# AndreasKarg/raytracer-weekend

Measured on AMD Instinct MI355X. Metric: Mrays/sec at 1920x1080, 512 spp, 50 bounces; 1/2/4/8-GPU scaling, higher is better.
Workload: dtype f32; 1 GPU; Random-spheres scene, 1920x1080, 512 spp, 1xMI355X (configs[1]); scene=jumpy-balls, width=1920, height=1080, spp=512, max_depth=50, rays_per_frame=3103484398, tiles=32400, launches_per_frame=1, parallelism=tiles1

## Files before the change

include/rtw.h:

```cpp
#ifndef RTW_H
#define RTW_H
#include <stddef.h>
#include <stdint.h>

#ifdef __cplusplus
extern "C" {
#endif

#define RTW_ABI_VERSION 7

enum {
  RTW_OK = 0,
  RTW_EINVAL = -22,
  RTW_ENOMEM = -12,
  RTW_ENODEV = -19,
  RTW_ESTATE = -71,
  RTW_EIO = -5
};

typedef struct rtw_scene rtw_scene;

typedef struct {
  float origin[3], lower_left_corner[3], horizontal[3], vertical[3];
  float u[3], v[3], w[3];
// ... 91 lines not shown
int rtw_progress_decode(const uint8_t* frame, size_t len, rtw_progress_msg* msg);

int rtw_render_device(rtw_scene* s, int device, const rtw_camera* cam, const float background[3],
                      uint32_t w, uint32_t h, uint32_t spp, uint32_t max_depth, uint64_t seed,
                      const uint32_t* d_tile_ids, uint32_t n_tiles, float* d_out, void* stream,
                      uint32_t flags, rtw_stats* stats);
int rtw_render_device_strided(rtw_scene* s, int device, const rtw_camera* cam, const float background[3],
                              uint32_t w, uint32_t h, uint32_t spp, uint32_t max_depth, uint64_t seed,
                              uint32_t first_tile, uint32_t tile_stride, uint32_t n_tiles, float* d_out,
                              void* stream, uint32_t flags, rtw_stats* stats);
typedef struct {
  float origin[3], direction[3];
  float time;
  uint32_t reserved;
  uint64_t stream;
} rtw_ray;
typedef struct {
  float p[3], normal[3];
  float t, u, v;
  uint32_t material, key, flags;
} rtw_hit;
enum {
  RTW_HIT_HIT = 1,
  RTW_HIT_FRONT_FACE = 2,
  RTW_HIT_BAD_RAY = 4
};
int rtw_hit_rays(rtw_scene* s, int device, uint64_t n, const void* rays, void* hits, rtw_stats* stats);
int rtw_hit_rays_device(rtw_scene* s, int device, uint64_t n, const void* d_rays, void* d_hits, void* stream,
                        rtw_stats* stats);

typedef struct {
  float attenuation[3];
  float emitted[3];
  uint32_t flags, reserved;
} rtw_scatter;
enum {
  RTW_SCATTER_SCATTERED = 1,
  RTW_SCATTER_MISS = 2,
  RTW_SCATTER_BAD = 4
};
int rtw_camera_rays(rtw_scene* s, int device, const rtw_camera* cam, uint32_t w, uint32_t h, uint32_t spp,
                    uint64_t seed, uint64_t first, uint64_t n, void* rays, rtw_stats* stats);
int rtw_camera_rays_device(rtw_scene* s, int device, const rtw_camera* cam, uint32_t w, uint32_t h, uint32_t spp,
                           uint64_t seed, uint64_t first, uint64_t n, void* d_rays, void* stream, rtw_stats* stats);
int rtw_scatter_rays(rtw_scene* s, int device, uint64_t n, const void* rays, const void* hits,
                     const float background[3], void* out_rays, void* out_scatter, rtw_stats* stats);
int rtw_scatter_rays_device(rtw_scene* s, int device, uint64_t n, const void* d_rays, const void* d_hits,
                            const float background[3], void* d_out_rays, void* d_out_scatter, void* stream,
                            rtw_stats* stats);

typedef struct {
  float color[3];
  uint32_t segments;
  uint64_t stream;
  uint32_t flags, reserved;
} rtw_sample;
enum { RTW_SAMPLE_END_MISS = 1, RTW_SAMPLE_END_NO_SCATTER = 2 ,
       RTW_SAMPLE_BAD_RAY = 4, RTW_SAMPLE_END_DEPTH = 8 };
int rtw_sample_rays(rtw_scene* s, int device, uint64_t n, const void* rays, const float background[3],
                    uint32_t max_depth, void* samples, rtw_stats* stats);
int rtw_sample_rays_device(rtw_scene* s, int device, uint64_t n, const void* d_rays, const float background[3],
                           uint32_t max_depth, void* d_samples, void* stream, rtw_stats* stats);

int rtw_render_status(rtw_scene* s, int device);
int rtw_diag_corrupt_bvh(rtw_scene* s, int device);
int rtw_diag_alias_devices(rtw_scene* s, int n);

int rtw_render_multi(rtw_scene* s, int n_gpus, const rtw_camera* cam, const float background[3], uint32_t w,
                     uint32_t h, uint32_t spp, uint32_t max_depth, uint64_t seed, float* out_rgb_sum,
                     rtw_stats* stats);
int rtw_render_multi_times(const rtw_scene* s, float* device_ms, uint32_t cap, float* gather_ms);

int rtw_tile_partition(uint32_t w, uint32_t h, uint32_t n_parts, uint32_t part, uint32_t* ids, uint32_t cap,
                       uint32_t* n_ids);

int rtw_unpack_tiles_device(int device, uint32_t w, uint32_t h, const uint32_t* d_tile_ids,
                            uint32_t n_tiles, const float* d_packed, float* d_image, void* stream);

int rtw_path_kernel_times(rtw_scene* s, int device, float* ms, uint32_t max_n);

int rtw_diag_libm(int fn, uint32_t n, const float* a, const float* b, float* out);
int rtw_diag_sweep(int fn, uint32_t lo, uint32_t hi, uint64_t* counts, uint32_t* bad, uint32_t cap);
int rtw_diag_recip(uint32_t n, const float* b, float* out);

int rtw_tonemap(const float* rgb_sum, uint32_t n_pixels, uint32_t spp, uint8_t* rgb8);

int rtw_scene_preset(rtw_scene* s, const char* name, float aspect_ratio, uint64_t seed,
                     const char* models_dir, rtw_camera* cam, float background[3]);
int rtw_preset_cameras(const char* name, float aspect_ratio, const char* models_dir, rtw_camera* cams,
                       uint32_t cap, uint32_t* n);

int rtw_scene_dump(const rtw_scene* s, char* buf, size_t cap, size_t* needed);
int rtw_scene_image(const rtw_scene* s, uint32_t k, const uint8_t** rgb8, uint32_t* w, uint32_t* h);
int64_t rtw_scene_info(const rtw_scene* s, int what);
int rtw_scene_nodes(const rtw_scene* s, const void** nodes, uint32_t* n_nodes);
int rtw_scene_nodes_half(const rtw_scene* s, const void** nodes, uint32_t* n_nodes);

#ifdef __cplusplus
}
#endif
#endif
```

raytracer-weekend_amd/__init__.py:

```python
from __future__ import annotations

import contextlib
import ctypes as C
import os
from pathlib import Path

import numpy as np

PKG_DIR = Path(__file__).resolve().parent
REPO_ROOT = PKG_DIR.parent
LIB_PATH = Path(os.environ.get("RTW_LIB_PATH") or PKG_DIR / "lib" / "librtw_amd.so")
MODELS_DIR = REPO_ROOT / "models"

RTW_EINVAL, RTW_ENOMEM, RTW_ENODEV, RTW_ESTATE, RTW_EIO = -22, -12, -19, -71, -5
FLAG_COUNT_TRAVERSAL = 1
NO_MATERIAL = 0xFFFFFFFF


class RtwError(RuntimeError):
    def __init__(self, code: int, msg: str):
        super().__init__(f"rtw error {code}: {msg}")
        self.code = code


# ... 66 lines not shown
                      ("v", np.float32), ("material", np.uint32), ("key", np.uint32), ("flags", np.uint32)])
MSG_IMAGE_START, MSG_PIXEL, MSG_IMAGE_END = 0, 1, 2
PIXEL_SINK = C.CFUNCTYPE(C.c_int, C.POINTER(rtw_pixel), C.c_uint32, C.c_void_p)
PIXEL_DTYPE = np.dtype([("row", np.uint32), ("column", np.uint32), ("color", np.float32, 3)])

_F = C.POINTER(C.c_float)
_U32 = C.POINTER(C.c_uint32)
_U8 = C.POINTER(C.c_uint8)
_SIGS = {
    "rtw_last_error": (C.c_char_p, []),
    "rtw_abi_version": (C.c_int, []),
    "rtw_device_count": (C.c_int, []),
    "rtw_scene_create": (C.c_int, [C.POINTER(C.c_void_p)]),
    "rtw_scene_destroy": (None, [C.c_void_p]),
    "rtw_texture_solid": (C.c_int, [C.c_void_p, C.c_float, C.c_float, C.c_float, _U32]),
    "rtw_texture_checker": (C.c_int, [C.c_void_p, C.c_uint32, C.c_uint32, C.c_float, _U32]),
    "rtw_texture_image": (C.c_int, [C.c_void_p, _U8, C.c_uint32, C.c_uint32, _U32]),
    "rtw_texture_uvdebug": (C.c_int, [C.c_void_p, _U32]),
    "rtw_texture_noise": (C.c_int, [C.c_void_p, _F, _U32, C.c_float, _U32]),
    "rtw_perlin_generate": (C.c_int, [C.c_uint64, _F, _U32]),
    "rtw_material_isotropic": (C.c_int, [C.c_void_p, C.c_uint32, _U32]),
    "rtw_material_lambertian": (C.c_int, [C.c_void_p, C.c_uint32, _U32]),
    "rtw_material_metal": (C.c_int, [C.c_void_p, C.c_float, C.c_float, C.c_float, C.c_float, _U32]),
    "rtw_material_dielectric": (C.c_int, [C.c_void_p, C.c_float, _U32]),
    "rtw_material_diffuse_light": (C.c_int, [C.c_void_p, C.c_uint32, _U32]),
    "rtw_begin_list": (C.c_int, [C.c_void_p]),
    "rtw_begin_bvh": (C.c_int, [C.c_void_p, C.c_float, C.c_float]),
    "rtw_begin_translate": (C.c_int, [C.c_void_p, C.c_float, C.c_float, C.c_float]),
    "rtw_begin_rotate_y": (C.c_int, [C.c_void_p, C.c_float]),
    "rtw_begin_constant_medium": (C.c_int, [C.c_void_p, C.c_float, C.c_uint32, _U32]),
    "rtw_end": (C.c_int, [C.c_void_p]),
    "rtw_add_spheres": (C.c_int, [C.c_void_p, C.c_uint32, _F, _F, _F, _F, _U32]),
    "rtw_add_moving_spheres": (C.c_int, [C.c_void_p, C.c_uint32] + [_F] * 9 + [_U32]),
    "rtw_add_rects": (C.c_int, [C.c_void_p, C.c_uint32, _U32, _F, _F, _F, _F, _F, _U32]),
    "rtw_add_cuboid": (C.c_int, [C.c_void_p, _F, _F, C.c_uint32]),
    "rtw_add_triangles": (C.c_int, [C.c_void_p, C.c_uint32, _F, _F, _U8, _F, _U8, C.c_uint32]),
    "rtw_load_wavefront_obj": (C.c_int, [C.c_void_p, C.c_char_p, C.c_void_p, C.c_uint32, _U32]),
    "rtw_scene_commit": (C.c_int, [C.c_void_p, C.c_int]),
    "rtw_camera_new": (C.c_int, [_F, _F, _F, C.c_float, C.c_float, C.c_float, C.c_float, C.c_float,
                                 C.c_float, C.POINTER(rtw_camera)]),
    "rtw_render": (C.c_int, [C.c_void_p, C.POINTER(rtw_camera), _F, C.c_uint32, C.c_uint32, C.c_uint32,
                             C.c_uint32, C.c_uint64, _F, C.POINTER(rtw_stats)]),
    "rtw_render_device": (C.c_int, [C.c_void_p, C.c_int, C.POINTER(rtw_camera), _F, C.c_uint32, C.c_uint32,
                                    C.c_uint32, C.c_uint32, C.c_uint64, _U32, C.c_uint32, C.c_void_p,
                                    C.c_void_p, C.c_uint32, C.POINTER(rtw_stats)]),
    "rtw_render_device_strided": (C.c_int, [C.c_void_p, C.c_int, C.POINTER(rtw_camera), _F, C.c_uint32,
                                            C.c_uint32, C.c_uint32, C.c_uint32, C.c_uint64, C.c_uint32, C.c_uint32,
                                            C.c_uint32, C.c_void_p, C.c_void_p, C.c_uint32, C.POINTER(rtw_stats)]),
    "rtw_hit_rays": (C.c_int, [C.c_void_p, C.c_int, C.c_uint64, C.POINTER(rtw_ray), C.POINTER(rtw_hit),
                               C.POINTER(rtw_stats)]),
    "rtw_hit_rays_device": (C.c_int, [C.c_void_p, C.c_int, C.c_uint64, C.c_void_p, C.c_void_p, C.c_void_p,
                                      C.POINTER(rtw_stats)]),
    "rtw_camera_rays": (C.c_int, [C.c_void_p, C.c_int, C.POINTER(rtw_camera), C.c_uint32, C.c_uint32, C.c_uint32,
                                  C.c_uint64, C.c_uint64, C.c_uint64, C.POINTER(rtw_ray), C.POINTER(rtw_stats)]),
    "rtw_camera_rays_device": (C.c_int, [C.c_void_p, C.c_int, C.POINTER(rtw_camera), C.c_uint32, C.c_uint32,
                                         C.c_uint32, C.c_uint64, C.c_uint64, C.c_uint64, C.c_void_p, C.c_void_p,
                                         C.POINTER(rtw_stats)]),
    "rtw_scatter_rays": (C.c_int, [C.c_void_p, C.c_int, C.c_uint64, C.POINTER(rtw_ray), C.POINTER(rtw_hit), _F,
                                   C.POINTER(rtw_ray), C.POINTER(rtw_scatter), C.POINTER(rtw_stats)]),
    "rtw_scatter_rays_device": (C.c_int, [C.c_void_p, C.c_int, C.c_uint64, C.c_void_p, C.c_void_p, _F, C.c_void_p,
                                          C.c_void_p, C.c_void_p, C.POINTER(rtw_stats)]),
    "rtw_sample_rays": (C.c_int, [C.c_void_p, C.c_int, C.c_uint64, C.POINTER(rtw_ray), _F, C.c_uint32,
                                  C.POINTER(rtw_sample), C.POINTER(rtw_stats)]),
    "rtw_sample_rays_device": (C.c_int, [C.c_void_p, C.c_int, C.c_uint64, C.c_void_p, _F, C.c_uint32, C.c_void_p,
                                         C.c_void_p, C.POINTER(rtw_stats)]),
    "rtw_render_status": (C.c_int, [C.c_void_p, C.c_int]),
    "rtw_diag_corrupt_bvh": (C.c_int, [C.c_void_p, C.c_int]),
    "rtw_diag_alias_devices": (C.c_int, [C.c_void_p, C.c_int]),
    "rtw_path_kernel_times": (C.c_int, [C.c_void_p, C.c_int, _F, C.c_uint32]),
    "rtw_render_multi": (C.c_int, [C.c_void_p, C.c_int, C.POINTER(rtw_camera), _F, C.c_uint32, C.c_uint32,
                                   C.c_uint32, C.c_uint32, C.c_uint64, _F, C.POINTER(rtw_stats)]),
    "rtw_render_multi_times": (C.c_int, [C.c_void_p, _F, C.c_uint32, _F]),
    "rtw_tile_partition": (C.c_int, [C.c_uint32, C.c_uint32, C.c_uint32, C.c_uint32, _U32, C.c_uint32, _U32]),
    "rtw_render_stream": (C.c_int, [C.c_void_p, C.POINTER(rtw_camera), _F, C.c_uint32, C.c_uint32, C.c_uint32,
                                    C.c_uint32, C.c_uint64, C.c_uint32, PIXEL_SINK, C.c_void_p,
                                    C.POINTER(rtw_stats)]),
    "rtw_progress_encode": (C.c_int, [C.POINTER(rtw_progress_msg), _U8, C.c_size_t, C.POINTER(C.c_size_t)]),
    "rtw_progress_decode": (C.c_int, [_U8, C.c_size_t, C.POINTER(rtw_progress_msg)]),
    "rtw_unpack_tiles_device": (C.c_int, [C.c_int, C.c_uint32, C.c_uint32, C.c_void_p, C.c_uint32,
                                          C.c_void_p, C.c_void_p, C.c_void_p]),
    "rtw_tonemap": (C.c_int, [_F, C.c_uint32, C.c_uint32, _U8]),
    "rtw_diag_libm": (C.c_int, [C.c_int, C.c_uint32, _F, _F, _F]),
    "rtw_diag_recip": (C.c_int, [C.c_uint32, _F, _F]),
    "rtw_diag_sweep": (C.c_int, [C.c_int, C.c_uint32, C.c_uint32, C.POINTER(C.c_uint64), _U32, C.c_uint32]),
    "rtw_scene_preset": (C.c_int, [C.c_void_p, C.c_char_p, C.c_float, C.c_uint64, C.c_char_p,
                                   C.POINTER(rtw_camera), _F]),
    "rtw_preset_cameras": (C.c_int, [C.c_char_p, C.c_float, C.c_char_p, C.POINTER(rtw_camera), C.c_uint32,
                                     _U32]),
    "rtw_scene_dump": (C.c_int, [C.c_void_p, C.c_char_p, C.c_size_t, C.POINTER(C.c_size_t)]),
    "rtw_scene_image": (C.c_int, [C.c_void_p, C.c_uint32, C.POINTER(_U8), _U32, _U32]),
    "rtw_scene_nodes": (C.c_int, [C.c_void_p, C.POINTER(C.c_void_p), _U32]),
    "rtw_scene_nodes_half": (C.c_int, [C.c_void_p, C.POINTER(C.c_void_p), _U32]),
    "rtw_scene_info": (C.c_int64, [C.c_void_p, C.c_int]),
}
EXPORTED_SYMBOLS = tuple(_SIGS)

_lib = None


ABI_VERSION = 7


def lib_sha() -> str:
    import hashlib
    return hashlib.sha256(LIB_PATH.read_bytes()).hexdigest()[:16] if LIB_PATH.exists() else ""


def lib() -> C.CDLL:
    global _lib
    if _lib is None:
        if not LIB_PATH.exists():
            raise RtwError(RTW_ENODEV, f"{LIB_PATH} not built (run __graft_entry__.build())")
        try:
            import torch
        except ImportError:
            pass
        L = C.CDLL(str(LIB_PATH))
        for name, (res, args) in _SIGS.items():
            fn = getattr(L, name)
            fn.restype = res
            fn.argtypes = args
        if L.rtw_abi_version() != ABI_VERSION:
            raise RtwError(RTW_ESTATE, f"{LIB_PATH} has ABI {L.rtw_abi_version()}, this mirror {ABI_VERSION}")
        _lib = L
    return _lib


def _check(rc: int) -> None:
    if rc != 0:
        raise RtwError(rc, lib().rtw_last_error().decode())


def _fa(x) -> np.ndarray:
    return np.ascontiguousarray(np.asarray(x, dtype=np.float32).reshape(-1))


def _ua(x) -> np.ndarray:
    return np.ascontiguousarray(np.asarray(x, dtype=np.uint32).reshape(-1))


def _fp(a: np.ndarray):
    return a.ctypes.data_as(_F)


def _up(a: np.ndarray):
    return a.ctypes.data_as(_U32)


def device_count() -> int:
    return int(lib().rtw_device_count())


class Camera:

    def __init__(self, c: rtw_camera):
        self.c = c

    @classmethod
    def new(cls, look_from, look_at, vup, vfov, aspect, aperture, focus_dist, time0=0.0, time1=1.0):
        c = rtw_camera()
        _check(lib().rtw_camera_new(_fp(_fa(look_from)), _fp(_fa(look_at)), _fp(_fa(vup)), vfov, aspect,
                                    aperture, focus_dist, time0, time1, C.byref(c)))
        return cls(c)

    def as_dict(self) -> dict:
        return {k: (list(getattr(self.c, k)) if k not in ("lens_radius", "time0", "time1")
# ... 342 lines not shown
            self.seed, first_tile, tile_stride, n_tiles, C.c_void_p(d_out_ptr), C.c_void_p(stream_ptr), flags,
            C.byref(st) if want_stats else None))
        return st.as_dict() if want_stats else None


def make_rays(origins, directions, times=None, streams=None) -> np.ndarray:
    o = np.asarray(origins, np.float32).reshape(-1, 3)
    rays = np.zeros(len(o), RAY_DTYPE)
    rays["origin"] = o
    rays["direction"] = np.asarray(directions, np.float32).reshape(-1, 3)
    if times is not None:
        rays["time"] = np.asarray(times, np.float32).reshape(-1)
    if streams is not None:
        rays["stream"] = np.asarray(streams, np.uint64).reshape(-1)
    return rays


def progress_encode(kind: int, width=0, height=0, spp=0, pixel=None) -> bytes:
    m = rtw_progress_msg(kind=kind, width=width, height=height, samples_per_pixel=spp)
    if pixel is not None:
        m.pixel.row, m.pixel.column = int(pixel[0]), int(pixel[1])
        m.pixel.color[:] = [float(x) for x in pixel[2]]
    out = (C.c_uint8 * 64)()
    n = C.c_size_t()
    _check(lib().rtw_progress_encode(C.byref(m), out, 64, C.byref(n)))
    return bytes(out[:n.value])


def progress_decode(frame: bytes) -> dict:
    buf = (C.c_uint8 * max(1, len(frame))).from_buffer_copy(frame or b"\0")
    m = rtw_progress_msg()
    _check(lib().rtw_progress_decode(buf, len(frame), C.byref(m)))
    d = {"kind": int(m.kind)}
    if m.kind == MSG_IMAGE_START:
        d.update(width=int(m.width), height=int(m.height), samples_per_pixel=int(m.samples_per_pixel))
    elif m.kind == MSG_PIXEL:
        d.update(row=int(m.pixel.row), column=int(m.pixel.column), color=[float(x) for x in m.pixel.color])
    return d


def perlin_generate(seed: int = 0):
    g = np.zeros(768, np.float32)
    p = np.zeros(768, np.uint32)
    _check(lib().rtw_perlin_generate(seed, _fp(g), _up(p)))
    return g.reshape(256, 3), p.reshape(3, 256)


def preset_cameras(name: str, aspect: float, models_dir=None) -> list:
    n = C.c_uint32()
    md = str(models_dir or MODELS_DIR).encode()
    _check(lib().rtw_preset_cameras(name.encode(), aspect, md, None, 0, C.byref(n)))
    cams = (rtw_camera * max(1, n.value))()
    _check(lib().rtw_preset_cameras(name.encode(), aspect, md, cams, n.value, C.byref(n)))
    return [Camera(cams[k]) for k in range(n.value)]


def unpack_tiles_device(w, h, d_tiles_ptr, n_tiles, d_packed_ptr, d_image_ptr, device=-1, stream_ptr=0):
    _check(lib().rtw_unpack_tiles_device(device, w, h, C.c_void_p(d_tiles_ptr), n_tiles, C.c_void_p(d_packed_ptr),
                                         C.c_void_p(d_image_ptr), C.c_void_p(stream_ptr)))


def diag_libm(fn: int, a, b=None) -> np.ndarray:
    a = _fa(a)
    bb = _fa(b) if b is not None else None
    out = np.empty_like(a)
    _check(lib().rtw_diag_libm(fn, len(a), _fp(a), _fp(bb) if bb is not None else None, _fp(out)))
    return out


def diag_sweep(fn: int, lo: int = 0, hi: int = 0xFFFFFFFF, cap: int = 64):
    counts = (C.c_uint64 * 2)()
    bad = np.zeros(max(1, cap), np.uint32)
    _check(lib().rtw_diag_sweep(fn, lo, hi, counts, _up(bad), cap))
    return int(counts[0]), int(counts[1]), bad[:min(cap, int(counts[0]))]


def diag_recip(b) -> np.ndarray:
    b = _fa(b)
    out = np.empty_like(b)
    _check(lib().rtw_diag_recip(len(b), _fp(b), _fp(out)))
    return out


def tile_partition(w: int, h: int, n_parts: int, part: int):
    nt = n_tiles(w, h)
    per = (nt + n_parts - 1) // n_parts if n_parts > 0 else 0
    ids = np.zeros(max(1, per), np.uint32)
    n = C.c_uint32()
    _check(lib().rtw_tile_partition(w, h, n_parts, part, _up(ids), per, C.byref(n)))
    return ids[:per], int(n.value)


def n_tiles(w: int, h: int) -> int:
    return ((w + 7) // 8) * ((h + 7) // 8)


def tonemap(sums: np.ndarray, spp: int) -> np.ndarray:
    s = np.ascontiguousarray(sums, np.float32)
    out = np.empty(s.shape, np.uint8)
    _check(lib().rtw_tonemap(_fp(s.reshape(-1)), s.size // 3, spp, out.ctypes.data_as(_U8)))
    return out


def image_height(width: int, aspect: float = 1.7777778) -> int:
    import math
    x = width / aspect
    return int(math.floor(x + 0.5))


def camera_aspect(width: int, height: int) -> float:
    return float(np.float32(width) / np.float32(height))
```

raytracer-weekend_amd/csrc/rtw.hpp:

```cpp
#pragma once
#include <stdexcept>
#include <string>
#include <vector>

#include "../../include/rtw.h"

namespace rtw {

struct Error : std::runtime_error {
  int code;
  Error(int c, const char* m) : std::runtime_error(m), code(c) {}
};
inline void check(int rc) {
  if (rc != RTW_OK) throw Error(rc, rtw_last_error());
}

struct Vec3 {
  float x, y, z;
};
using Point3 = Vec3;
using Color = Vec3;

struct Pixel {
  uint32_t row, column;
// ... 59 lines not shown
  World& operator=(const World&) = delete;
  rtw_scene* raw() const { return s_; }

  TextureId solid_rgb(float r, float g, float b) { TextureId t; check(rtw_texture_solid(s_, r, g, b, &t)); return t; }
  TextureId checker(TextureId odd, TextureId even, float freq) { TextureId t; check(rtw_texture_checker(s_, odd, even, freq, &t)); return t; }
  TextureId image(const uint8_t* rgb, uint32_t w, uint32_t h) { TextureId t; check(rtw_texture_image(s_, rgb, w, h, &t)); return t; }
  TextureId uv_debug() { TextureId t; check(rtw_texture_uvdebug(s_, &t)); return t; }
  TextureId noise(float scale, uint64_t perlin_seed) {
    float g[768];
    uint32_t p[768];
    check(rtw_perlin_generate(perlin_seed, g, p));
    TextureId t;
    check(rtw_texture_noise(s_, g, p, scale, &t));
    return t;
  }

  MaterialId lambertian(TextureId t) { MaterialId m; check(rtw_material_lambertian(s_, t, &m)); return m; }
  MaterialId lambertian_solid(Color c) { return lambertian(solid_rgb(c.x, c.y, c.z)); }
  MaterialId metal(Color albedo, float fuzz) { MaterialId m; check(rtw_material_metal(s_, albedo.x, albedo.y, albedo.z, fuzz, &m)); return m; }
  MaterialId dielectric(float ir) { MaterialId m; check(rtw_material_dielectric(s_, ir, &m)); return m; }
  MaterialId diffuse_light(TextureId t) { MaterialId m; check(rtw_material_diffuse_light(s_, t, &m)); return m; }
  MaterialId isotropic(TextureId t) { MaterialId m; check(rtw_material_isotropic(s_, t, &m)); return m; }

  void sphere(Point3 c, float r, MaterialId m) { check(rtw_add_spheres(s_, 1, &c.x, &c.y, &c.z, &r, &m)); }
  void moving_sphere(Point3 c0, float t0, Point3 c1, float t1, float r, MaterialId m) {
    check(rtw_add_moving_spheres(s_, 1, &c0.x, &c0.y, &c0.z, &t0, &c1.x, &c1.y, &c1.z, &t1, &r, &m));
  }
  void rect(uint32_t axis, float a0, float a1, float b0, float b1, float k, MaterialId m) {
    check(rtw_add_rects(s_, 1, &axis, &a0, &a1, &b0, &b1, &k, &m));
  }
  void xy_rect(float x0, float x1, float y0, float y1, float k, MaterialId m) { rect(0, x0, x1, y0, y1, k, m); }
  void xz_rect(float x0, float x1, float z0, float z1, float k, MaterialId m) { rect(1, x0, x1, z0, z1, k, m); }
  void yz_rect(float y0, float y1, float z0, float z1, float k, MaterialId m) { rect(2, y0, y1, z0, z1, k, m); }
  void cuboid(Point3 p0, Point3 p1, MaterialId m) {
    const float a[3] = {p0.x, p0.y, p0.z}, b[3] = {p1.x, p1.y, p1.z};
    check(rtw_add_cuboid(s_, a, b, m));
  }
  void triangle(const Point3 v[3], MaterialId m) {
    const float f[9] = {v[0].x, v[0].y, v[0].z, v[1].x, v[1].y, v[1].z, v[2].x, v[2].y, v[2].z};
    check(rtw_add_triangles(s_, 1, f, nullptr, nullptr, nullptr, nullptr, m));
  }
  uint32_t load_wavefront_obj(const std::string& path, uint32_t material_override = UINT32_MAX) {
    uint32_t n = 0;
    check(rtw_load_wavefront_obj(s_, path.c_str(), nullptr, material_override, &n));
    return n;
  }
  template <class F> void list(F&& body) { check(rtw_begin_list(s_)); body(); check(rtw_end(s_)); }
  template <class F> void bvh(float t0, float t1, F&& body) { check(rtw_begin_bvh(s_, t0, t1)); body(); check(rtw_end(s_)); }
  template <class F> void translate(Vec3 off, F&& body) { check(rtw_begin_translate(s_, off.x, off.y, off.z)); body(); check(rtw_end(s_)); }
  template <class F> void rotate_y(float deg, F&& body) { check(rtw_begin_rotate_y(s_, deg)); body(); check(rtw_end(s_)); }
  template <class F> void constant_medium(float density, TextureId t, F&& body) {
    check(rtw_begin_constant_medium(s_, density, t, nullptr)); body(); check(rtw_end(s_));
  }

  void preset(const std::string& name, float aspect, uint64_t seed, const std::string& models, Camera& cam, Color& bg) {
    float b[3];
    check(rtw_scene_preset(s_, name.c_str(), aspect, seed, models.c_str(), &cam.c, b));
    bg = Color{b[0], b[1], b[2]};
  }
  static std::vector<Camera> preset_cameras(const std::string& name, float aspect, const std::string& models) {
    uint32_t n = 0;
    check(rtw_preset_cameras(name.c_str(), aspect, models.c_str(), nullptr, 0, &n));
    std::vector<rtw_camera> raw(n);
    check(rtw_preset_cameras(name.c_str(), aspect, models.c_str(), raw.data(), n, &n));
    std::vector<Camera> out(n);
    for (uint32_t k = 0; k < n; ++k) out[k].c = raw[k];
    return out;
  }
  void commit(int device = -1) { check(rtw_scene_commit(s_, device)); }
  std::vector<Hit> hit_rays(const std::vector<Ray>& rays, int device = -1, rtw_stats* st = nullptr) const {
    std::vector<Hit> hits(rays.size());
    check(rtw_hit_rays(s_, device, rays.size(), rays.data(), hits.data(), st));
    return hits;
  }
  std::vector<Ray> camera_rays(const Camera& cam, uint32_t w, uint32_t h, uint32_t spp, uint64_t seed,
                               uint64_t first = 0, uint64_t n = UINT64_MAX, int device = -1,
                               rtw_stats* st = nullptr) const {
    const uint64_t paths = (uint64_t)w * h * spp;
    if (n == UINT64_MAX) n = first <= paths ? paths - first : 0;
    std::vector<Ray> rays(n);
    check(rtw_camera_rays(s_, device, &cam.c, w, h, spp, seed, first, n, rays.data(), st));
    return rays;
  }
  std::vector<Scatter> scatter_rays(std::vector<Ray>& rays, const std::vector<Hit>& hits, Color background,
                                    int device = -1, rtw_stats* st = nullptr) const {
    if (rays.size() != hits.size()) throw Error(RTW_EINVAL, "rays and hits differ in length");
    std::vector<Scatter> sc(rays.size());
    const float bg[3] = {background.x, background.y, background.z};
    check(rtw_scatter_rays(s_, device, rays.size(), rays.data(), hits.data(), bg, rays.data(), sc.data(), st));
    return sc;
  }
  std::vector<Sample> sample_rays(const std::vector<Ray>& rays, Color background, uint32_t max_depth = 50,
                                  int device = -1, rtw_stats* st = nullptr) const {
    std::vector<Sample> out(rays.size());
    const float bg[3] = {background.x, background.y, background.z};
    check(rtw_sample_rays(s_, device, rays.size(), rays.data(), bg, max_depth, out.data(), st));
    return out;
  }

 private:
  rtw_scene* s_ = nullptr;
};

class Raytracer {
 public:
  Raytracer(World& world, const Camera& cam, Color background, uint32_t w, uint32_t h, uint32_t spp,
            uint64_t seed = 0, uint32_t max_depth = 50)
      : world_(world), cam_(cam), bg_(background), w_(w), h_(h), spp_(spp), seed_(seed), depth_(max_depth) {}

  std::vector<float> render_sums(rtw_stats* st = nullptr) const {
    std::vector<float> out((size_t)w_ * h_ * 3);
    const float bg[3] = {bg_.x, bg_.y, bg_.z};
    check(rtw_render(world_.raw(), &cam_.c, bg, w_, h_, spp_, depth_, seed_, out.data(), st));
    return out;
  }
  std::vector<Pixel> render(rtw_stats* st = nullptr) const {
    std::vector<float> s = render_sums(st);
    std::vector<Pixel> px;
    px.reserve((size_t)w_ * h_);
    for (uint32_t r = 0; r < h_; ++r)
      for (uint32_t i = 0; i < w_; ++i) {
        const float* c = &s[((size_t)r * w_ + i) * 3];
        px.push_back(Pixel{h_ - 1 - r, i, Color{c[0], c[1], c[2]}});
      }
    return px;
  }

 private:
  World& world_;
  Camera cam_;
  Color bg_;
  uint32_t w_, h_, spp_;
  uint64_t seed_;
  uint32_t depth_;
};

}
```

raytracer-weekend_amd/csrc/rtw_capi.cpp:

```cpp
#include <math.h>
#include <stdarg.h>
#include <stdio.h>
#include <stdlib.h>
#include <string.h>

#include <mutex>
#include <new>
#include <set>
#include <string>
#include <vector>

#include "../../include/rtw.h"
#include "rtw_scene.hpp"

namespace rtw {

static thread_local char g_err[512];

int fail(int code, const char* fmt, ...) {
  va_list ap;
  va_start(ap, fmt);
  vsnprintf(g_err, sizeof g_err, fmt, ap);
  va_end(ap);
  return code;
// ... 474 lines not shown
    for (uint8_t k = 1; k < code; ++k) {
      if (i >= n) return fail(RTW_EIO, "COBS: truncated block");
      raw.push_back(f[i++]);
    }
    if (code != 0xFF && i < n) raw.push_back(0);
  }
  size_t at = 0;
  auto varint = [&](uint32_t* v) -> bool {
    uint32_t x = 0;
    for (int sh = 0; sh < 35; sh += 7) {
      if (at >= raw.size()) return false;
      const uint8_t b = raw[at++];
      x |= (uint32_t)(b & 0x7F) << sh;
      if (!(b & 0x80)) { *v = x; return true; }
    }
    return false;
  };
  auto f32 = [&](float* v) -> bool {
    if (at + 4 > raw.size()) return false;
    uint32_t b = 0;
    for (int k = 0; k < 4; ++k) b |= (uint32_t)raw[at++] << (8 * k);
    memcpy(v, &b, 4);
    return true;
  };
  memset(m, 0, sizeof *m);
  if (!varint(&m->kind)) return fail(RTW_EIO, "postcard: unexpected end (DeserializeUnexpectedEnd)");
  bool ok = true;
  if (m->kind == RTW_MSG_IMAGE_START) ok = varint(&m->width) && varint(&m->height) && varint(&m->samples_per_pixel);
  else if (m->kind == RTW_MSG_PIXEL)
    ok = varint(&m->pixel.row) && varint(&m->pixel.column) && f32(&m->pixel.color[0]) && f32(&m->pixel.color[1]) &&
         f32(&m->pixel.color[2]);
  else if (m->kind != RTW_MSG_IMAGE_END) return fail(RTW_EIO, "postcard: bad enum tag %u", m->kind);
  if (!ok) return fail(RTW_EIO, "postcard: unexpected end (DeserializeUnexpectedEnd)");
  return RTW_OK;
}

int rtw_scene_dump(const rtw_scene* s, char* buf, size_t cap, size_t* needed) {
  if (!s) return fail(RTW_EINVAL, "scene is NULL");
  std::string t = dump_scene(s->s);
  if (needed) *needed = t.size() + 1;
  if (buf && cap >= t.size() + 1) memcpy(buf, t.c_str(), t.size() + 1);
  else if (buf) return fail(RTW_EINVAL, "buffer too small (%zu < %zu)", cap, t.size() + 1);
  return RTW_OK;
}
int rtw_scene_image(const rtw_scene* s, uint32_t k, const uint8_t** px, uint32_t* w, uint32_t* h) {
  if (!s || !px || !w || !h) return fail(RTW_EINVAL, "NULL argument");
  uint32_t seen = 0;
  for (const TexH& t : s->s.tex) {
    if (t.type != TT_IMAGE) continue;
    if (seen++ == k) { *px = t.img.data(); *w = t.w; *h = t.h; return RTW_OK; }
  }
  return fail(RTW_EINVAL, "no image texture #%u", k);
}
int rtw_scene_nodes(const rtw_scene* s, const void** nodes, uint32_t* n_nodes) {
  if (!s || !nodes || !n_nodes) return fail(RTW_EINVAL, "NULL argument");
  *nodes = s->s.flat.nodes4.empty() ? nullptr : (const void*)s->s.flat.nodes4.data();
  *n_nodes = (uint32_t)s->s.flat.nodes4.size();
  return RTW_OK;
}
int rtw_scene_nodes_half(const rtw_scene* s, const void** nodes, uint32_t* n_nodes) {
  if (!s || !nodes || !n_nodes) return fail(RTW_EINVAL, "NULL argument");
  *nodes = s->s.flat.nodes4h.empty() ? nullptr : (const void*)s->s.flat.nodes4h.data();
  *n_nodes = (uint32_t)s->s.flat.nodes4h.size();
  return RTW_OK;
}
int64_t rtw_scene_info(const rtw_scene* s, int what) {
  if (!s) return -1;
  const Scene& sc = s->s;
  switch (what) {
    case 1: return (int64_t)sc.mat.size();
    case 2: return (int64_t)sc.tex.size();
    case 3: return (int64_t)sc.flat.nodes4.size();
    case 7: return (int64_t)sc.flat.nodes.size();
    case 8: return (int64_t)sc.flat.stack_need;
    case 9: return (int64_t)sc.flat.features;
    case 10: return (int64_t)sc.flat.perlins.size();
    case 11: return (int64_t)sc.flat.stack_need4;
    case 12: return (int64_t)sc.flat.lgroups.size();
    case 13: return (int64_t)sc.flat.rect_fast;
    case 14: return (int64_t)sc.flat.far_check;
    case 15: return (int64_t)llround(1000.0 * (double)sc.flat.far_d0);
    case 16: case 17: case 18: case 19: case 20: case 21: case 22: case 23:
      return selected_kernel_info(sc, what - 16);
    case 4: return (int64_t)sc.flat.depth;
    case 5: return (int64_t)sc.flat.always.size();
    case 6: return (int64_t)sc.flat.insts.size();
    default: {
      if (sc.committed) return (int64_t)sc.flat.prims.size();
      int64_t n = 0;
      std::vector<uint32_t> todo{0};
      while (!todo.empty()) {
        const Node& nd = sc.nodes[todo.back()];
        todo.pop_back();
        if (nd.kind == NK_CUBOID) n += 6;
        else if (nd.kind == NK_MEDIUM || nd.kind >= NK_SPHERE) n += 1;
        else todo.insert(todo.end(), nd.ch.begin(), nd.ch.end());
      }
      return n;
    }
  }
}

}
```

raytracer-weekend_amd/csrc/rtw_dev_trace.hpp:

```cpp
#pragma once
#include "rtw_dev_hit.hpp"

namespace rtw {
namespace dev {

struct TraceState {
  Best b;
  int32_t node;
  int32_t pend;
  int32_t sp;
  bool on;
};

template <int AXIS, bool FAST>
__device__ __forceinline__ void rect_list_test(const Ray& lr, V3 y, float4 q0, float k, uint32_t pi, float& bt,
                                               int32_t& bp) {
  const float o_k = AXIS == 0 ? lr.o.z : (AXIS == 1 ? lr.o.y : lr.o.x);
  const float d_k = AXIS == 0 ? lr.d.z : (AXIS == 1 ? lr.d.y : lr.d.x);
  const float y_k = AXIS == 0 ? y.z : (AXIS == 1 ? y.y : y.x);
  const float o_a = AXIS == 2 ? lr.o.y : lr.o.x, d_a = AXIS == 2 ? lr.d.y : lr.d.x;
  const float o_b = AXIS == 0 ? lr.o.y : lr.o.z, d_b = AXIS == 0 ? lr.d.y : lr.d.z;
  const float num = k - o_k;
  bool acc;
  if constexpr (FAST) {
// ... 113 lines not shown
  const float dd = fabsf(d) > 1e-20f ? d : copysignf(1e-20f, d);
  return __builtin_amdgcn_rcpf(dd);
}
__device__ __forceinline__ float cull_tmax(float t) { return __builtin_fmaf(t, 1.0e-5f, t) + 1.0e-5f; }
template <bool COUNT, uint32_t FEAT, int STACK, int BLK, bool C16, int NCAP>
__device__ void trace_far(const DevScene& S, const Ray& r, Best& b, float delta, uint16_t* stk16, int32_t* stk,
                          uint32_t* cnt, uint64_t seg, uint32_t* err, const float4* lnodes) {
  const DevFar* const FR = far_record(S);
  const char* const NB = NCAP > 0 ? reinterpret_cast<const char*>(lnodes)
                                  : reinterpret_cast<const char*>(S.prims) - uload(&FR->nodes_back);
  const uint32_t n_bvh = uload(&FR->n_bvh);
  const V3 inv = mk(cull_inv(r.d.x), cull_inv(r.d.y), cull_inv(r.d.z));
  const V3 ood = mk(r.o.x * inv.x, r.o.y * inv.y, r.o.z * inv.z);
  const V3 bn = mk(-ood.x - delta * fabsf(inv.x), -ood.y - delta * fabsf(inv.y), -ood.z - delta * fabsf(inv.z));
  const V3 bf = mk(-ood.x + delta * fabsf(inv.x), -ood.y + delta * fabsf(inv.y), -ood.z + delta * fabsf(inv.z));
  const uint32_t nx = inv.x < 0.f ? 16u : 0u, ny = (inv.y < 0.f ? 16u : 0u) + 32u, nz = (inv.z < 0.f ? 16u : 0u) + 64u;
  const uint32_t fx = nx ^ 16u, fy = ny ^ 16u, fz = nz ^ 16u;
  int32_t node = 0, sp = 0;
  bool over = false;
  for (uint32_t guard = 0;; ++guard) {
    if (node < 0) {
      if (sp == 0) break;
      --sp;
      node = C16 ? (int32_t)stk16[sp * BLK] : stk[sp * BLK];
    }
    if (guard >= (1u << 20)) {
      *err = 1u;
      b.prim = -2;
      return;
    }
    if (COUNT) cnt[0]++;
    const uint32_t nb = (uint32_t)node << 7;
    const float4 qnx = *reinterpret_cast<const float4*>(NB + (nb + nx)), qfx = *reinterpret_cast<const float4*>(NB + (nb + fx));
    const float4 qny = *reinterpret_cast<const float4*>(NB + (nb + ny)), qfy = *reinterpret_cast<const float4*>(NB + (nb + fy));
    const float4 qnz = *reinterpret_cast<const float4*>(NB + (nb + nz)), qfz = *reinterpret_cast<const float4*>(NB + (nb + fz));
    const uint4 cw = *reinterpret_cast<const uint4*>(NB + (nb + (C16 ? 112u : 96u)));
    const float tmax_c = cull_tmax(b.t);
    const float NX[4] = {qnx.x, qnx.y, qnx.z, qnx.w}, FX[4] = {qfx.x, qfx.y, qfx.z, qfx.w};
    const float NY[4] = {qny.x, qny.y, qny.z, qny.w}, FY[4] = {qfy.x, qfy.y, qfy.z, qfy.w};
    const float NZ[4] = {qnz.x, qnz.y, qnz.z, qnz.w}, FZ[4] = {qfz.x, qfz.y, qfz.z, qfz.w};
    const uint32_t W[4] = {cw.x, cw.y, cw.z, cw.w};
    uint32_t hits = 0;
    float tnear = INFINITY;
    int kn = -1;
#pragma unroll
    for (int k = 0; k < 4; ++k) {
      const float tn = fmaxf(fmaxf(fmaxf(__builtin_fmaf(NX[k], inv.x, bn.x), __builtin_fmaf(NY[k], inv.y, bn.y)),
                                   __builtin_fmaf(NZ[k], inv.z, bn.z)), 0.0f);
      const float tf = fminf(fminf(fminf(__builtin_fmaf(FX[k], inv.x, bf.x), __builtin_fmaf(FY[k], inv.y, bf.y)),
                                   __builtin_fmaf(FZ[k], inv.z, bf.z)), tmax_c);
      const bool h = W[k] != 0u && tn <= tf;
      hits |= h ? 1u << k : 0u;
      const bool inner = C16 ? (W[k] & 0x8000u) == 0u : (int32_t)W[k] >= 0;
      const bool nearer = h && inner && tn < tnear;
      tnear = nearer ? tn : tnear;
      kn = nearer ? k : kn;
    }
    node = kn < 0 ? -1 : (int32_t)(kn == 0 ? W[0] : (kn == 1 ? W[1] : (kn == 2 ? W[2] : W[3])));
    hits &= kn < 0 ? hits : ~(1u << kn);
    while (hits) {
      const int k = __builtin_ctz(hits);
      hits &= hits - 1u;
      const uint32_t w = k == 0 ? W[0] : (k == 1 ? W[1] : (k == 2 ? W[2] : W[3]));
      if (C16 ? (w & 0x8000u) != 0u : (int32_t)w < 0) {
        const uint32_t v = C16 ? w & 0xFFFFu : ~w;
        const uint32_t first = C16 ? (v >> 2) & 0x1FFFu : v >> 3, n = C16 ? (v & 3u) + 1u : v & 7u;
        for (uint32_t q = 0; q < n; ++q) test_prim<COUNT, FEAT>(S, first + q, r, b, cnt, seg);
      } else if (sp < STACK) {
        if constexpr (C16) stk16[sp * BLK] = (uint16_t)w;
        else stk[sp * BLK] = (int32_t)w;
        ++sp;
      } else {
        over = true;
      }
    }
  }
  if (over)
    for (uint32_t pi = 0; pi < n_bvh; ++pi) test_prim<COUNT, FEAT>(S, pi, r, b, cnt, seg);
}

constexpr bool far_kernel_feat(uint32_t feat) {
  return !(feat & F_LIST) && (feat & (F_SPHERE | F_MSPHERE | F_MEDIUM)) && feat != F_MESHES;
}
template <bool COUNT, uint32_t FEAT, int STACK = 1, int BLK = BLOCK, bool C16 = false, int NCAP = 0>
__device__ __forceinline__ void trace_begin(const DevScene& S, const Ray& r, TraceState& ts, uint32_t* cnt,
                                            uint64_t seg, uint16_t* stk16 = nullptr, int32_t* stk = nullptr,
                                            uint32_t* err = nullptr, const float4* lnodes = nullptr) {
  ts.b = Best{INFINITY, 0u, -1, 0.0f, 0.0f};
  constexpr bool RECT_LIST = (FEAT & F_LIST) && (FEAT & F_RECT) && !(FEAT & (F_SPHERE | F_MSPHERE | F_TRI | F_MEDIUM));
  if constexpr (RECT_LIST) {
    trace_rect_list<COUNT>(S, r, ts.b, cnt);
  } else if (FEAT & F_INST) {
    uint32_t cur = 0;
    Ray lr = r;
    const uint32_t a0 = S.n_prims - S.n_always;
    for (uint32_t k = 0; k < S.n_always; ++k) {
      const uint32_t pi = a0 + k;
      const uint32_t inst = uload(&S.prims[pi].type_inst) >> 8;
      if (inst != cur) {
        lr = inst ? to_local<true>(S.insts + inst, r) : r;
        cur = inst;
      }
      test_prim<COUNT, FEAT, true, true>(S, pi, lr, ts.b, cnt, seg);
    }
  } else {
    constexpr bool SPH_ONLY = (FEAT & (F_RECT | F_TRI | F_MEDIUM | F_INST)) == 0 && (FEAT & (F_SPHERE | F_MSPHERE));
    SphRcp rq;
    if constexpr (SPH_ONLY) rq = sph_rcp(r);
    for (uint32_t k = 0; k < S.n_always; ++k)
      test_prim<COUNT, FEAT, false, true>(S, uload(S.always + k), r, ts.b, cnt, seg, SPH_ONLY ? &rq : nullptr);
  }
  if constexpr ((FEAT & F_LIST) && !RECT_LIST) {
    const bool nan_hit = ts.b.prim >= 0 && (ts.b.prim & RECT_NAN_HIT) != 0;
    ts.b.t = nan_hit ? __builtin_nanf("") : ts.b.t;
    ts.b.prim = nan_hit ? (ts.b.prim & ~RECT_NAN_HIT) : ts.b.prim;
  }
  bool walk = true;
#if defined(RTW_DIAG_FAR)
  constexpr int DF = RTW_DIAG_FAR;
#else
  constexpr int DF = 0;
#endif
  constexpr bool FAR = DF != 1 && far_kernel_feat(FEAT);
  if constexpr (FAR) {
    if (S.far_check) {
      const float4* const FR = reinterpret_cast<const float4*>(far_record(S));
      const float4 mid = uload(FR), half = uload(FR + 1);
      const float tx = fabsf(r.o.x - mid.x) + half.x;
      const float ty = fabsf(r.o.y - mid.y) + half.y;
      const float tz = fabsf(r.o.z - mid.z) + half.z;
      const float D2 = tx * tx + ty * ty + tz * tz;
      const bool far = D2 > mid.w;
      if (__any(far)) {
        bool need = false;
        float delta = 0.0f;
        if (far && DF != 2) {
          const float4 lo = uload(FR + 2), hi = uload(FR + 3), e = uload(FR + 4);
          const float D = __builtin_amdgcn_sqrtf(D2) * 1.000001f;
          delta = fminf(half.w * D2 + lo.w, hi.w * D + e.x) + (e.y * D + e.z);
          const float ix = __builtin_amdgcn_rcpf(r.d.x), iy = __builtin_amdgcn_rcpf(r.d.y), iz = __builtin_amdgcn_rcpf(r.d.z);
          const float ox = r.o.x - mid.x, oy = r.o.y - mid.y, oz = r.o.z - mid.z;
          const float hx = half.x + delta, hy = half.y + delta, hz = half.z + delta;
          const float ax = (-hx - ox) * ix, bx = (hx - ox) * ix, ay = (-hy - oy) * iy, by = (hy - oy) * iy;
          const float az = (-hz - oz) * iz, bz = (hz - oz) * iz;
          const float tn = fmaxf(fmaxf(fminf(ax, bx), fminf(ay, by)), fmaxf(fminf(az, bz), 0.0f));
          const float tf = fminf(fminf(fmaxf(ax, bx), fmaxf(ay, by)),
                                 fminf(fmaxf(az, bz), cull_tmax(ts.b.t)));
          need = tn <= tf;
        }
        walk = !far;
        if (DF == 5) asm volatile("" ::"v"((uint32_t)need));
        if (DF != 3 && DF != 5 && __builtin_expect(__any(need), 0))
          if (need) trace_far<COUNT, FEAT, STACK, BLK, C16, NCAP>(S, r, ts.b, delta, stk16, stk, cnt, seg, err, lnodes);
      }
    }
  }
  int32_t root = S.n_nodes ? 0 : -1;
  if constexpr ((FEAT & F_TRI) != 0) {
    root = __builtin_amdgcn_readfirstlane(root);
    asm volatile("" : "+s"(root));
  } else {
    asm volatile("" : "+v"(root));
  }
  ts.node = walk ? root : -1;
  ts.pend = 0;
  ts.sp = 0;
  ts.on = true;
}

#ifndef RTW_MESH_ROOT
#define RTW_MESH_ROOT 5
#endif
#ifndef REGEN_RING
#define REGEN_RING 2
#endif
#ifndef REGEN_RING_LDSN
#define REGEN_RING_LDSN 8
#endif
typedef _Float16 half2_t __attribute__((ext_vector_type(2)));
__device__ __forceinline__ half2_t as_h2(uint32_t u) { return __builtin_bit_cast(half2_t, u); }

template <bool COUNT, int STACK, bool SPILL, uint32_t FEAT, int BLK, int NCAP, bool HN = false, bool S16 = false>
__device__ void trace_run(const DevScene& S, const Ray& r, TraceState& ts, int32_t* stk, int32_t* spill,
                          uint32_t spill_lanes, uint32_t* cnt, uint32_t quota, uint32_t leaf_thr, uint64_t seg,
                          uint32_t* err, uint64_t* tph, const float4* lnodes, uint16_t* stk16) {
  constexpr bool K16 = NCAP > 0;
  constexpr bool CODES = K16 || HN || S16;
  constexpr bool SPH_ONLY = (FEAT & (F_RECT | F_TRI | F_MEDIUM | F_INST)) == 0 && (FEAT & (F_SPHERE | F_MSPHERE));
  SphRcp rq;
  if constexpr (SPH_ONLY) rq = sph_rcp(r);
  Ray tri_ray = r;
  if constexpr ((FEAT & F_TRI) != 0) {
    if (S.bvh_tri && (FEAT & F_INST) && S.tri_inst) {
      if (S.tri_inst == S.uni_inst) tri_ray.o = sub(r.o, mk(S.uni_off[0], S.uni_off[1], S.uni_off[2]));
      else tri_ray = to_local<true>(S.insts + S.tri_inst, r);
    }
  }
  uint64_t tm = COUNT ? __builtin_amdgcn_s_memtime() : 0;
  if constexpr (NCAP == 0) __builtin_amdgcn_s_setprio(2);
  auto tick = [&](int k) {
    if (COUNT) {
      const uint64_t t = __builtin_amdgcn_s_memtime();
      tph[k] += t - tm;
      tm = t;
    }
  };
  const V3 inv = mk(cull_inv(r.d.x), cull_inv(r.d.y), cull_inv(r.d.z));
  const V3 ood = mk(r.o.x * inv.x, r.o.y * inv.y, r.o.z * inv.z);
  const uint32_t nx = inv.x < 0.f ? 16u : 0u, ny = (inv.y < 0.f ? 16u : 0u) + 32u, nz = (inv.z < 0.f ? 16u : 0u) + 64u;
  const uint32_t fx = nx ^ 16u, fy = ny ^ 16u, fz = nz ^ 16u;
  const char* const NB = NCAP > 0 ? reinterpret_cast<const char*>(lnodes)
                                  : (HN ? reinterpret_cast<const char*>(S.hnodes) : reinterpret_cast<const char*>(S.nodes));
  constexpr bool ROOT = HN && S16 && NCAP == 0 && RTW_MESH_ROOT > 0;
  constexpr int32_t NROOT = RTW_MESH_ROOT;
#pragma unroll
  for (int lv = 0; lv < (ROOT ? (NROOT > 1 ? 2 : 1) : 0); ++lv) {
    if (__any(ts.node >= 0 && ts.node < NROOT)) {
      if (ts.node >= 0 && ts.node < NROOT) {
        const char* const TB = reinterpret_cast<const char*>(lnodes) + (uint32_t)ts.node * 112u;
        const uint4 px = *reinterpret_cast<const uint4*>(TB + nx);
        const uint4 py = *reinterpret_cast<const uint4*>(TB + ny);
        const uint4 pz = *reinterpret_cast<const uint4*>(TB + nz);
        const uint4 cq = *reinterpret_cast<const uint4*>(TB + 96u);
        const half2_t oxy = as_h2(cq.z), oz = as_h2(cq.w);
        const V3 bs = mk(__builtin_fmaf((float)oxy.x, inv.x, -ood.x), __builtin_fmaf((float)oxy.y, inv.y, -ood.y),
                         __builtin_fmaf((float)oz.x, inv.z, -ood.z));
        const uint32_t PQ[3][4] = {{px.x, px.y, px.z, px.w}, {py.x, py.y, py.z, py.w}, {pz.x, pz.y, pz.z, pz.w}};
        float NA[3][4], FA[3][4];
#pragma unroll
        for (int q = 0; q < 3; ++q) {
          const half2_t n01 = as_h2(PQ[q][0]), n23 = as_h2(PQ[q][1]), f01 = as_h2(PQ[q][2]), f23 = as_h2(PQ[q][3]);
          NA[q][0] = (float)n01.x; NA[q][1] = (float)n01.y; NA[q][2] = (float)n23.x; NA[q][3] = (float)n23.y;
          FA[q][0] = (float)f01.x; FA[q][1] = (float)f01.y; FA[q][2] = (float)f23.x; FA[q][3] = (float)f23.y;
        }
        const int32_t CW[4] = {(int32_t)(int16_t)(cq.x & 0xFFFFu), (int32_t)cq.x >> 16, (int32_t)(int16_t)(cq.y & 0xFFFFu),
                               (int32_t)cq.y >> 16};
        if (COUNT) {
          cnt[0]++;
          cnt[14] += (CW[0] != 0) + (CW[1] != 0) + (CW[2] != 0) + (CW[3] != 0);
        }
        const float tmax_c = cull_tmax(ts.b.t);
        int32_t next = -1, bk = -1;
        float best = INFINITY;
        bool hit[4];
#pragma unroll
        for (int k = 0; k < 4; ++k) {
          const float a0 = __builtin_fmaf(NA[0][k], inv.x, bs.x), b0 = __builtin_fmaf(NA[1][k], inv.y, bs.y);
// ... 238 lines not shown
```

raytracer-weekend_amd/csrc/rtw_device.hpp:

```cpp
#pragma once
#include <stdint.h>

namespace rtw {

enum PrimType : uint32_t {
  PT_SPHERE = 0,
  PT_MSPHERE = 1,
  PT_RECT_XY = 2,
  PT_RECT_XZ = 3,
  PT_RECT_YZ = 4,
  PT_TRI = 5,
  PT_MEDIUM = 6,
};

struct alignas(16) DevPrim {
  float q0[4], q1[4], q2[4];
  uint32_t type_inst;
  uint32_t key;
  uint32_t mat;
  uint32_t aux;
};
static_assert(sizeof(DevPrim) == 64, "DevPrim must be 64 B");

struct alignas(16) DevGroup {
// ... 94 lines not shown
constexpr uint32_t F_ALL = ((1u << 16) - 1) | F_TEXGEN;
constexpr uint32_t F_LIST = 1u << 16;
constexpr uint32_t F_SPHERES = F_SPHERE | F_MSPHERE | F_CHECKER | F_LAMBERT | F_METAL | F_DIEL | F_LIGHT;
constexpr uint32_t F_BOXES = F_RECT | F_INST | F_LAMBERT | F_METAL | F_DIEL | F_LIGHT;
constexpr uint32_t F_SMOKE = F_BOXES | F_MEDIUM | F_ISO;
constexpr uint32_t F_MESHES = F_SPHERE | F_RECT | F_TRI | F_INST | F_CHECKER | F_IMAGE | F_LAMBERT | F_LIGHT | F_TEXGEN;

struct DevScene {
  const DevNode4* nodes;
  const DevNode4h* hnodes;
  const DevPrim* prims;
  const uint32_t* always;
  const DevTriShade* tshade;
  const DevInst* insts;
  const DevMat* mats;
  const DevTex* texs;
  const uint8_t* texels;
  const DevPerlin* perlins;
  const DevShade* shade;
  const DevGroup* lgroups;
  uint32_t n_nodes, n_prims, n_always, n_insts;
  uint32_t n_lgroups;
  uint32_t msphere_unit;
  uint32_t uni_inst;
  float uni_off[3];
  uint32_t rect_fast;
  uint32_t bvh_tri;
  uint32_t tri_inst;
  uint32_t far_check;
};

struct alignas(16) DevFar {
  float mid[3], d2;
  float half[3], q;
  float lo[3], q0;
  float hi[3], s;
  float s0, l, l0;
  uint32_t n_bvh;
  uint32_t nodes_back;
  uint32_t pad[2];
};
static_assert(sizeof(DevFar) == 96, "DevFar must be 96 B");

constexpr uint32_t DEVFAR_BACK = 256;

constexpr uint32_t DISP = 8;
constexpr uint32_t DISP_STRIDE = 16;
constexpr uint32_t COUNTER_WORDS = 32 + DISP * DISP_STRIDE;

struct DevCamera {
  float origin[3], llc[3], horizontal[3], vertical[3], u[3], v[3];
  float lens_radius, time0, time1;
};

struct RenderArgs {
  DevScene scene;
  DevCamera cam;
  float bg[3];
  uint32_t w, h, spp, max_depth;
  uint32_t tiles_x;
  uint32_t slot_base;
  uint32_t quota16;
  uint32_t leaf16;
  uint32_t regen_min;
  uint32_t batch;
  uint64_t spp_magic;
  float fw1, fh1;
  float rw1, rh1;
  float time_span;
  uint64_t tiles_x_magic;
  const uint32_t* tile_ids;
  uint32_t tile_first, tile_stride;
  uint32_t packed_out;
  uint64_t seed_hash;
  uint64_t n_paths;
  float* sbuf;
  float* out;
  unsigned long long* counters;
  unsigned long long* queue;
  uint32_t* err;
  int32_t* spill;
  uint32_t spill_depth;
  uint32_t spill_lanes;
};

}
```

raytracer-weekend_amd/csrc/rtw_flatten.cpp:

```cpp
#include <math.h>

#include <cmath>
#include <stdlib.h>
#include <string.h>

#include <algorithm>
#include <map>
#include <vector>

#include "../../include/rtw.h"
#include "rtw_scene.hpp"

namespace rtw {
namespace {

struct Box {
  float lo[3] = {INFINITY, INFINITY, INFINITY};
  float hi[3] = {-INFINITY, -INFINITY, -INFINITY};
  void grow(const float p[3]) {
    for (int a = 0; a < 3; ++a) { lo[a] = fminf(lo[a], p[a]); hi[a] = fmaxf(hi[a], p[a]); }
  }
  void grow(const Box& b) {
    for (int a = 0; a < 3; ++a) { lo[a] = fminf(lo[a], b.lo[a]); hi[a] = fmaxf(hi[a], b.hi[a]); }
  }
// ... 628 lines not shown
      for (int k = 0; k < 256; ++k) {
        for (int a = 0; a < 3; ++a) P.g[k][a] = t.grad[3 * k + a];
        for (int a = 0; a < 3; ++a) P.perm[a][k] = (uint8_t)t.perm[256 * a + k];
      }
      f.perlins.push_back(P);
    }
    f.texs.push_back(d);
  }
  if (f.texels.empty()) f.texels.resize(4, 0);
  if (f.perlins.empty()) f.perlins.resize(1);
  if (f.mats.empty()) f.mats.push_back(DevMat{});
  if (f.texs.empty()) f.texs.push_back(DevTex{});

  DevInst ident;
  memset(&ident, 0, sizeof ident);
  f.insts.push_back(ident);

  Builder B(s, f);
  std::vector<uint32_t> chain;
  B.walk(0, chain);
  if (B.err) return B.err;
  if (B.leaves.size() >= (1u << 31)) return fail(RTW_EINVAL, "too many primitives");

  std::vector<Leaf> huge, rest;
  uint32_t list_max = 32;
  if (const char* e = tuning_env("RTW_LIST_MAX")) list_max = (uint32_t)std::min(64, std::max(0, atoi(e)));
  if (B.leaves.size() <= list_max) {
    huge = B.leaves;
  } else if (B.leaves.size() > 16) {
    std::vector<float> d;
    for (const Leaf& L : B.leaves) d.push_back(L.wbox.diag());
    std::vector<float> sorted = d;
    size_t q = (size_t)(0.95 * (sorted.size() - 1));
    std::nth_element(sorted.begin(), sorted.begin() + q, sorted.end());
    float thr = 20.f * sorted[q];
    size_t nh = 0;
    for (float x : d) nh += x > thr;
    for (size_t k = 0; k < B.leaves.size(); ++k)
      ((nh <= 8 && d[k] > thr) ? huge : rest).push_back(B.leaves[k]);
  } else {
    rest = B.leaves;
  }

  {
    size_t ntri = 0;
    uint32_t inst = UINT32_MAX;
    bool one_inst = true;
    for (const Leaf& L : rest)
      if ((L.p.type_inst & 0xffu) == PT_TRI) {
        ++ntri;
        const uint32_t i = L.p.type_inst >> 8;
        if (inst == UINT32_MAX) inst = i;
        one_inst = one_inst && i == inst;
      }
    const char* knob = tuning_env("RTW_TRI_LEAF");
    if ((!knob || atoi(knob)) && ntri > 16 && one_inst && rest.size() - ntri <= 4 &&
        huge.size() + (rest.size() - ntri) <= 8) {
      std::vector<Leaf> tris;
      for (const Leaf& L : rest) ((L.p.type_inst & 0xffu) == PT_TRI ? tris : huge).push_back(L);
      rest.swap(tris);
      f.bvh_tri = 1;
      f.tri_inst = inst;
    }
  }
  far_bound(rest, f);
  if (!rest.empty()) {
    uint32_t lg = 0;
    while ((1ull << lg) < rest.size()) ++lg;
    BvhBuild bb{rest, f.nodes, lg + 4 < MAX_DEPTH ? MAX_DEPTH - lg - 1 : 3};
    Ref root = bb.build(0, (uint32_t)rest.size(), 0);
    if (root.count > 0) {
      DevNode nd;
      for (int a = 0; a < 3; ++a) {
        nd.b0lo[a] = root.box.lo[a]; nd.b0hi[a] = root.box.hi[a];
        nd.b1lo[a] = INFINITY; nd.b1hi[a] = -INFINITY;
      }
      nd.c0 = root.idx; nd.n0 = root.count;
      nd.c1 = -1; nd.n1 = 0;
      f.nodes.push_back(nd);
    }
    f.depth = bb.max_depth;
  }
  for (const Leaf& L : rest) f.prims.push_back(L.p);
  for (const Leaf& L : huge) {
    f.always.push_back((uint32_t)f.prims.size());
    f.prims.push_back(L.p);
  }
  if (f.depth > MAX_DEPTH) return fail(RTW_EINVAL, "BVH deeper than the traversal stack (%u)", f.depth);
  if (f.nodes.empty())
    for (size_t k = 1; k < f.always.size(); ++k)
      if (!(f.prims[f.always[k]].key > f.prims[f.always[k - 1]].key))
        return fail(RTW_EINVAL, "internal: list-mode prims out of key order");
  if (!f.tshade.empty()) {
    std::vector<DevTriShade> by_prim(f.prims.size());
    memset(by_prim.data(), 0, by_prim.size() * sizeof(DevTriShade));
    for (size_t k = 0; k < f.prims.size(); ++k)
      if ((f.prims[k].type_inst & 0xffu) == PT_TRI) {
        by_prim[k] = f.tshade[f.prims[k].aux];
        f.prims[k].aux = (uint32_t)k;
      }
    f.tshade.swap(by_prim);
  }
  f.rect_fast = 1;
  for (const DevPrim& p : f.prims) {
    const uint32_t t = p.type_inst & 0xffu;
    if ((t == PT_RECT_XY || t == PT_RECT_XZ || t == PT_RECT_YZ) &&
        !(fabsf(p.q1[0]) < 0x1p62f && p.q0[0] <= p.q0[1] && p.q0[2] <= p.q0[3] && std::isfinite(p.q0[0]) &&
          std::isfinite(p.q0[1]) && std::isfinite(p.q0[2]) && std::isfinite(p.q0[3])))
      f.rect_fast = 0;
  }
  for (size_t k = 0; k < f.always.size(); ++k) {
    const DevPrim& p = f.prims[f.always[k]];
    const uint32_t inst = p.type_inst >> 8, type = p.type_inst & 0xffu;
    if (!f.lgroups.empty() && f.lgroups.back().inst == inst && f.lgroups.back().type == type &&
        f.lgroups.back().first + f.lgroups.back().count == f.always[k])
      ++f.lgroups.back().count;
    else
      f.lgroups.push_back(DevGroup{f.always[k], 1u, inst, type});
  }
  {
    std::vector<DevGroup> g2;
    for (size_t g = 0; g < f.lgroups.size(); ++g) {
      const DevGroup& a = f.lgroups[g];
      if (g + 2 < f.lgroups.size()) {
        const DevGroup &b = f.lgroups[g + 1], &c = f.lgroups[g + 2];
        if (a.type == PT_RECT_XY && b.type == PT_RECT_XZ && c.type == PT_RECT_YZ && a.count == 2u && b.count == 2u &&
            c.count == 2u && a.inst == b.inst && b.inst == c.inst && b.first == a.first + 2u && c.first == b.first + 2u) {
          g2.push_back(DevGroup{a.first, 6u, a.inst, GK_BOX6});
          g += 2;
          continue;
        }
      }
      g2.push_back(a);
    }
    f.lgroups.swap(g2);
  }
  for (DevPrim& p : f.prims) {
    const uint32_t t = p.type_inst & 0xffu;
    if (t == PT_SPHERE || t == PT_MSPHERE) memcpy(&p.q1[3], &p.key, sizeof p.key);
  }
  f.mshade.clear();
  for (const DevMat& m : f.mats) f.mshade.push_back(shade_record(f, m));
  for (const DevPrim& p : f.prims) {
    const DevShade& d = f.mshade[p.mat];
    f.shade.push_back(d);
    if (((d.kind >> 8) & 0xfu) == SM_GENERIC) f.features |= F_TEXGEN;
  }
  if (!f.nodes.empty()) {
    if (rest.size() >= (1u << 28)) return fail(RTW_EINVAL, "too many BVH primitives for leaf words");
    Collapse col{f.nodes, f.nodes4};
    uint32_t bound = 0, bound4 = 0;
    col.build(0, &bound, &bound4);
    f.stack_need4 = bound4;
    if (f.nodes4.size() >= (1u << 25)) return fail(RTW_EINVAL, "BVH4 too large for 32-bit node offsets");
    f.stack_need = bound;
    if (f.stack_need > 4096) return fail(RTW_EINVAL, "BVH4 stack bound %u is unreasonable", f.stack_need);
    std::vector<uint8_t> seen4(f.nodes4.size(), 0), seenp(rest.size(), 0);
    std::vector<int32_t> todo{0};
    seen4[0] = 1;
    while (!todo.empty()) {
      const DevNode4 nd = f.nodes4[todo.back()];
      todo.pop_back();
      for (int k = 0; k < 4; ++k) {
        if (nd.lo_x[k] > nd.hi_x[k]) continue;
        const int32_t w = nd.child[k];
        if (w >= 0) {
// ... 105 lines not shown
```

raytracer-weekend_amd/csrc/rtw_kernel.hip:

```cpp
#include <hip/hip_runtime.h>
#include <math.h>
#include <stdio.h>
#include <stdlib.h>
#include <string.h>

#include <algorithm>

#include "../../include/rtw.h"
#include "rtw_scene.hpp"
#include "rtw_variants.hpp"
#include "rtw_shade_kernel.hpp"

namespace rtw {
namespace dev {

__global__ __launch_bounds__(256) void reduce_kernel(RenderArgs a, uint32_t n_slots) {
  const uint32_t g = blockIdx.x * blockDim.x + threadIdx.x;
  if (g >= n_slots * 64u) return;
  const uint32_t slot = g >> 6, l = g & 63u, gslot = a.slot_base + slot;
  const uint32_t tile = a.tile_ids ? a.tile_ids[gslot] : a.tile_first + gslot * a.tile_stride;
  const uint32_t i = (tile % a.tiles_x) * 8u + (l & 7u), row = (tile / a.tiles_x) * 8u + (l >> 3);
  if (i >= a.w || row >= a.h) return;
  float x = 0.f, y = 0.f, z = 0.f;
  const float* q = a.sbuf + ((size_t)slot * a.spp * 64u + l) * 3u;
  for (uint32_t s = 0; s < a.spp; ++s, q += 64u * 3u) {
#if RTW_NT_SAMPLES
    x = x + __builtin_nontemporal_load(q);
    y = y + __builtin_nontemporal_load(q + 1);
    z = z + __builtin_nontemporal_load(q + 2);
#else
    x = x + q[0];
    y = y + q[1];
    z = z + q[2];
#endif
  }
  float* o = a.packed_out ? a.out + ((size_t)gslot * 64u + l) * 3u : a.out + ((size_t)row * a.w + i) * 3u;
  o[0] = x;
  o[1] = y;
  o[2] = z;
}

__global__ void unpack_tiles_kernel(uint32_t w, uint32_t h, uint32_t tiles_x, const uint32_t* tiles,
                                    uint32_t n_tiles, const float* packed, float* img) {
  const uint32_t g = blockIdx.x * blockDim.x + threadIdx.x;
  if (g >= n_tiles * 64u) return;
  const uint32_t t = g >> 6, lane = g & 63u, tile = tiles[t];
  const uint32_t i = (tile % tiles_x) * 8u + (lane & 7u), row = (tile / tiles_x) * 8u + (lane >> 3);
  if (i >= w || row >= h) return;
  for (int c = 0; c < 3; ++c) img[((size_t)row * w + i) * 3 + c] = packed[(size_t)g * 3 + c];
}

__global__ void libm_kernel(int fn, uint32_t n, const float* a, const float* b, float* out) {
  const uint32_t g = blockIdx.x * blockDim.x + threadIdx.x;
  if (g >= n) return;
  const float x = a[g];
  if (fn == 4) {
    out[g] = div_by_recip(x, b[g], 1.0f / b[g]);
    return;
  }
  if (fn == 5) {
    out[g] = sqrt_rn(x);
    return;
  }
  out[g] = fn == 0 ? dev_log10f(x) : (fn == 1 ? dev_sinf(x) : (fn == 2 ? dev_acosf(x) : dev_atan2f(x, b[g])));
}

__global__ void sweep_kernel(int fn, uint32_t lo, uint32_t hi, unsigned long long* n, uint32_t* bad, uint32_t cap) {
  const uint64_t span = (uint64_t)hi - lo + 1u;
  const uint64_t stride = (uint64_t)gridDim.x * blockDim.x;
  unsigned long long nbad = 0, nskip = 0;
  for (uint64_t k = (uint64_t)blockIdx.x * blockDim.x + threadIdx.x; k < span; k += stride) {
    const uint32_t bits = lo + (uint32_t)k;
    const float b = __uint_as_float(bits);
    bool ok = true;
    if (fn == 0) {
      if (!rcp_rn_ok(b)) {
        ++nskip;
        continue;
      }
      const float f = rcp_rn_fast(b), r = 1.0f / b;
      ok = __float_as_uint(f) == __float_as_uint(r) || (f != f && r != r);
    }
    if (!ok) {
      const unsigned long long slot = atomicAdd(n + 2, 1ull);
      if (slot < cap) bad[slot] = bits;
      ++nbad;
    }
  }
  if (nbad) atomicAdd(n, nbad);
  if (nskip) atomicAdd(n + 1, nskip);
}

}

static uint64_t max_pass_paths(const Knobs& kn) {
  return 1ull << std::min(32, std::max(24, kn.pass_log2.get(32)));
}

static Knobs read_knobs() {
  auto knob = [](const char* name) {
    const char* e = tuning_env(name);
    return e ? Knob{true, atoi(e)} : Knob{};
  };
  Knobs k;
  k.stack_lds = knob("RTW_STACK_LDS");
  k.half_nodes = knob("RTW_HALF_NODES");
  k.generic = knob("RTW_GENERIC");
  k.list_all = knob("RTW_LIST_ALL");
  k.list_occ = knob("RTW_LIST_OCC");
  k.occ = knob("RTW_OCC");
  k.ldsn_waves = knob("RTW_LDSN_WAVES");
  k.lds_nodes = knob("RTW_LDS_NODES");
  k.ldsn_blk = knob("RTW_LDSN_BLK");
  k.mesh_s16 = knob("RTW_MESH_S16");
  k.batch = knob("RTW_BATCH");
  k.quota16 = knob("RTW_QUOTA16");
  k.leaf16 = knob("RTW_LEAF16");
  k.regen_min = knob("RTW_REGEN_MIN");
  k.pass_log2 = knob("RTW_PASS_LOG2");
  const char* v = getenv("RTW_VERBOSE");
  k.verbose = v && atoi(v);
  return k;
}

static Variant pick_kernel(const Knobs& kn, uint32_t feat, uint32_t need, bool list, uint32_t n_nodes, uint32_t need4,
                           bool codes16, bool has_half, bool far) {
  using namespace dev;
  if (kn.stack_lds.get(0) == 4) return make_variant<SPILL_TEST>();
  const bool sph = (feat & ~F_SPHERES) == 0;
  const int half_knob = kn.half_nodes.get(-1);
  const bool half = has_half && half_knob != 0;
  const bool half_lds = has_half && half_knob > 0;
  if (list) {
    if (kn.generic.get(0)) return make_variant<LIST_ALL>();
    if ((feat & ~F_BOXES) == 0 && !kn.list_all.get(0)) {
      if (kn.list_occ.get(8) == 6) return make_variant<LIST_BOXES6>();
      return make_variant<LIST_BOXES8>();
    }
    return make_variant<LIST_ALL>();
  }
  switch (kn.occ.get(sph ? 6 : 5)) {
    case 4: {
      const bool sp = need > (uint32_t)STACK_LDS;
      if (sph) return sp ? make_variant<with_spill(WALK4<F_SPHERES>)>() : make_variant<WALK4<F_SPHERES>>();
      return sp ? make_variant<with_spill(WALK4<F_ALL>)>() : make_variant<WALK4<F_ALL>>();
    }
    case 6: {
      const int ldsn_waves = kn.ldsn_waves.get(8);
      const bool ldsn = sph && codes16 && kn.lds_nodes.get(1);
      auto fits = [&](const KernelCfg& k) { return need4 <= (uint32_t)k.stack && n_nodes <= (uint32_t)k.ncap; };
      if (ldsn && ldsn_waves == 7 && fits(LDSN_448))
        return half_lds ? make_variant<with_half(LDSN_448)>() : make_variant<LDSN_448>();
      if (ldsn && ldsn_waves == 8 && fits(LDSN_1024) && !half_lds && kn.ldsn_blk.get(1024) == 1024)
        return make_variant<LDSN_1024>();
      if (ldsn && ldsn_waves == 8 && fits(LDSN_512))
        return half_lds ? make_variant<with_half(LDSN_512)>() : make_variant<LDSN_512>();
      if (ldsn && fits(LDSN_224))
        return half_lds ? make_variant<with_half(LDSN_224)>() : make_variant<LDSN_224>();
      if (sph && need <= (uint32_t)STACK_LDS5) return make_variant<SPHERES6>();
    }
      [[fallthrough]];
    default:
      if (kn.generic.get(0)) return pick5<F_ALL>(kn, need);
      if (sph) return pick5<F_SPHERES>(kn, need);
      if ((feat & ~F_BOXES) == 0) return pick5<F_BOXES>(kn, need);
      if ((feat & ~F_SMOKE) == 0) return pick5<F_SMOKE>(kn, need);
      if ((feat & ~F_MESHES) == 0) {
        if (far) return pick5<F_ALL>(kn, need);
        return pick_mesh(kn, need, half, codes16);
      }
      return pick5<F_ALL>(kn, need);
  }
}
static Variant path_kernel_variant(const Flat& f, const Knobs& kn) {
  const uint32_t feat = f.features, need = f.stack_need, need4 = f.stack_need4, nn = (uint32_t)f.nodes4.size();
  const bool list = f.nodes4.empty();
  const bool hh = f.codes16 && !f.nodes4h.empty();
  return pick_kernel(kn, feat, need, list, nn, need4, f.codes16, hh, f.far_check != 0);
}

int64_t selected_kernel_info(const Scene& s, int field) {
  const KernelCfg k = path_kernel_variant(s.flat, read_knobs()).cfg;
  const int64_t v[8] = {k.stack, k.spill, k.occ, k.feat, k.blk, k.ncap, k.half, k.s16};
  return field >= 0 && field < 8 ? v[field] : -1;
}

static int resident_blocks(DeviceCopy& c, GridSlot slot, const void* fn, int block, const char* what, bool verbose) {
  ResidentGrid& g = c.grids[slot];
  if (g.blocks > 0 && g.fn == fn) return g.blocks;
  int per_cu = 0, cus = 0;
  hipError_t e = hipOccupancyMaxActiveBlocksPerMultiprocessor(&per_cu, fn, block, 0);
  if (e != hipSuccess || per_cu < 1) per_cu = 1;
  if (hipDeviceGetAttribute(&cus, hipDeviceAttributeMultiprocessorCount, c.phys) != hipSuccess || cus < 1) cus = 256;
  g = ResidentGrid{fn, per_cu * cus};
  if (verbose)
    fprintf(stderr, "rtw: %s %p: block %d, %d resident blocks per CU x %d CUs\n", what, fn, block, per_cu, cus);
  return g.blocks;
}

template <class Kernel, class Args>
static int launch_query(Kernel kernel, const char* what, int resident, int block, uint64_t n, const Args& a,
                        hipStream_t stream, hipEvent_t ev0, hipEvent_t ev1) {
  const int grid = (int)std::min<uint64_t>((uint64_t)resident, (n + (uint32_t)block - 1u) / (uint32_t)block);
  if (ev0) HIPCHK(hipEventRecord(ev0, stream), "hipEventRecord");
  if (grid > 0) {
    hipLaunchKernelGGL(kernel, dim3(grid), dim3(block), 0, stream, a);
    HIPCHK(hipGetLastError(), what);
  }
  if (ev1) HIPCHK(hipEventRecord(ev1, stream), "hipEventRecord");
  return RTW_OK;
}

static uint32_t batch_ids(int v) { return (uint32_t)std::min(65536, std::max(64, v)) & ~63u; }

static unsigned long long* dispensers(const DeviceCopy& c) { return c.counters + 32; }

static RenderArgs frame_args(const DeviceCopy& c, const Frame& f, const TileSet& ts, float* d_out) {
  const rtw_camera* cam = f.cam;
  RenderArgs a;
  memset(&a, 0, sizeof a);
  a.scene = c.scene;
  memcpy(a.cam.origin, cam->origin, sizeof a.cam.origin);
  memcpy(a.cam.llc, cam->lower_left_corner, sizeof a.cam.llc);
  memcpy(a.cam.horizontal, cam->horizontal, sizeof a.cam.horizontal);
  memcpy(a.cam.vertical, cam->vertical, sizeof a.cam.vertical);
  memcpy(a.cam.u, cam->u, sizeof a.cam.u);
  memcpy(a.cam.v, cam->v, sizeof a.cam.v);
  a.cam.lens_radius = cam->lens_radius;
  a.cam.time0 = cam->time0;
  a.cam.time1 = cam->time1;
  memcpy(a.bg, f.bg, sizeof a.bg);
  a.w = f.w; a.h = f.h; a.spp = f.spp; a.max_depth = f.max_depth;
  a.tiles_x = f.tiles_x();
  a.spp_magic = f.spp > 1u ? UINT64_MAX / f.spp + 1u : 0u;
  a.fw1 = (float)(f.w - 1u);
  a.fh1 = (float)(f.h - 1u);
  a.rw1 = recip_rn(a.fw1);
  a.rh1 = recip_rn(a.fh1);
  {
    volatile float t0 = cam->time0, t1 = cam->time1;
    a.time_span = t1 - t0;
  }
  a.tiles_x_magic = a.tiles_x > 1u ? UINT64_MAX / a.tiles_x + 1u : 0u;
  a.tile_ids = ts.ids;
  a.tile_first = ts.first;
  a.tile_stride = ts.stride;
  a.packed_out = (ts.ids || ts.packed) ? 1u : 0u;
  a.err = c.err_host;
  uint64_t z = f.seed + 0x9E3779B97F4A7C15ull;
  z = (z ^ (z >> 30)) * 0xBF58476D1CE4E5B9ull;
  z = (z ^ (z >> 27)) * 0x94D049BB133111EBull;
  a.seed_hash = z ^ (z >> 31);
  a.out = d_out;
  a.counters = c.counters;
  a.queue = dispensers(c);
  return a;
}

struct WalkTuning {
  uint32_t leaf16, spill_depth, spill_lanes;
};
static WalkTuning tune_walk(const Knobs& kn, const Flat& flat, const KernelCfg& k, int grid) {
  WalkTuning t;
  const bool ldsn_spheres = k.lds_nodes() && flat.features == (flat.features & F_SPHERES);
  t.leaf16 = (uint32_t)std::min(16, std::max(1, kn.leaf16.get(ldsn_spheres ? 5 : 3)));
  const uint32_t lds = (uint32_t)k.stack;
  t.spill_depth = (!k.lds_nodes() && flat.stack_need > lds) ? flat.stack_need - lds : 0;
  t.spill_lanes = (uint32_t)grid * (uint32_t)k.blk;
  return t;
}

struct LaunchTuning {
  WalkTuning walk;
  uint32_t quota16, regen_min, batch;
};
static LaunchTuning tune_launch(const Knobs& kn, const Flat& flat, const KernelCfg& k, int grid) {
  LaunchTuning a;
  a.walk = tune_walk(kn, flat, k, grid);
  a.quota16 = (uint32_t)std::min(16, std::max(1, kn.quota16.get(12)));
  const bool small_batch = (k.lds_nodes() && k.blk == 1024) || flat.nodes4.empty();
  a.batch = batch_ids(kn.batch.get(small_batch ? 1024 : (int)dev::BATCH));
  const bool boxed = (flat.features & ~F_SMOKE) == 0;
  const int regen_dflt = k.ldsn_ring() ? REGEN_RING_LDSN : (k.sring() ? REGEN_RING : (boxed ? 8 : 24));
  a.regen_min = (uint32_t)std::min(64, std::max(1, kn.regen_min.get(regen_dflt)));
  return a;
}

static uint32_t pass_batch(uint32_t batch0, uint64_t n_paths, uint64_t waves) {
  const uint32_t batch_floor = batch0 >= 2048u ? 512u : 128u;
  uint32_t batch = batch0;
  while (batch / 2u >= batch_floor && n_paths < (uint64_t)batch * waves * 32u) batch /= 2u;
  return batch;
}

static int run_passes(Scene& sc, DeviceCopy& c, RenderArgs& a, const Knobs& kn, uint32_t n_slots, bool count,
                      hipStream_t stream) {
  const uint64_t per_slot = 64ull * a.spp;
  const uint32_t slots_per_pass = (uint32_t)std::max<uint64_t>(1, max_pass_paths(kn) / per_slot);
  const uint64_t need = std::min<uint64_t>(n_slots, slots_per_pass) * per_slot;
  if (int e = grow(c.sbuf, need * 3 * sizeof(float))) return e;
  a.sbuf = static_cast<float*>(c.sbuf.p);
  const Variant var = path_kernel_variant(sc.flat, kn);
  const KernelCfg& k = var.cfg;
  const int grid = resident_blocks(c, count ? GRID_PATH_COUNT : GRID_PATH, (const void*)var.fn[count], k.blk,
                                   "path kernel", kn.verbose);
  const LaunchTuning t = tune_launch(kn, sc.flat, k, grid);
  a.quota16 = t.quota16;
  a.leaf16 = t.walk.leaf16;
  a.regen_min = t.regen_min;
  a.spill_depth = t.walk.spill_depth;
  a.spill_lanes = t.walk.spill_lanes;
  if (int e = grow(c.spill, (size_t)a.spill_depth * a.spill_lanes * sizeof(int32_t))) return e;
  a.spill = static_cast<int32_t*>(c.spill.p);
  const uint64_t waves = (uint64_t)grid * (uint32_t)k.blk / 64u;
  for (uint32_t base = 0; base < n_slots; base += slots_per_pass) {
    const uint32_t ns = std::min(slots_per_pass, n_slots - base);
    a.slot_base = base;
    a.n_paths = (uint64_t)ns * per_slot;
    a.batch = kn.batch.set ? t.batch : pass_batch(t.batch, a.n_paths, waves);
    if (base) HIPCHK(hipMemsetAsync(a.queue, 0, DISP * DISP_STRIDE * sizeof(unsigned long long), stream),
                     "hipMemsetAsync(queue)");
    hipEvent_t* ke = c.kev[c.kev_head];
    if (int e = ensure_event(ke[0])) return e;
    if (int e = ensure_event(ke[1])) return e;
    HIPCHK(hipEventRecord(ke[0], stream), "hipEventRecord");
    hipLaunchKernelGGL(var.fn[count], dim3(grid), dim3(k.blk), 0, stream, a);
    HIPCHK(hipGetLastError(), "path_kernel launch");
    HIPCHK(hipEventRecord(ke[1], stream), "hipEventRecord");
    c.kev_head = (c.kev_head + 1) % 64u;
    c.kev_count = std::min(c.kev_count + 1u, 64u);
    hipLaunchKernelGGL(dev::reduce_kernel, dim3((ns * 64u + 255u) / 256u), dim3(256), 0, stream, a, ns);
    HIPCHK(hipGetLastError(), "reduce_kernel launch");
  }
  return RTW_OK;
}

int enqueue_render(Scene& sc, DeviceCopy& c, const Frame& f, const TileSet& ts, float* d_out, hipStream_t stream,
                   uint32_t flags, hipEvent_t ev0, hipEvent_t ev1) {
  if (int e = check_guard(c)) return e;
  if (int e = check_image_max(f.w, f.h)) return e;
  if (int e = check_shutter(*f.cam, sc.flat)) return e;
  RenderArgs a = frame_args(c, f, ts, d_out);
  const Knobs kn = read_knobs();
  HIPCHK(hipMemsetAsync(c.counters, 0, COUNTER_WORDS * sizeof(unsigned long long), stream), "hipMemsetAsync");
  if (ev0) HIPCHK(hipEventRecord(ev0, stream), "hipEventRecord");
  if (ts.n && (f.spp == 0 || f.max_depth == 0)) {
    size_t n = a.packed_out ? (size_t)ts.n * 64 * 3 : (size_t)f.w * f.h * 3;
    HIPCHK(hipMemsetAsync(d_out, 0, n * sizeof(float), stream), "hipMemsetAsync(out)");
  } else if (ts.n) {
    if (int e = run_passes(sc, c, a, kn, ts.n, flags & RTW_FLAG_COUNT_TRAVERSAL, stream)) return e;
  }
  if (ev1) HIPCHK(hipEventRecord(ev1, stream), "hipEventRecord");
  return RTW_OK;
}

int enqueue_hit_rays(Scene& sc, DeviceCopy& c, uint64_t n, const void* d_rays, void* d_hits, hipStream_t stream,
                     hipEvent_t ev0, hipEvent_t ev1) {
  const Knobs kn = read_knobs();
  const Variant var = path_kernel_variant(sc.flat, kn);
  const KernelCfg& k = var.cfg;
  const int resident = resident_blocks(c, GRID_HIT, (const void*)var.hit, k.blk, "query kernel", kn.verbose);
  const WalkTuning t = tune_walk(kn, sc.flat, k, resident);
  if (int e = grow(c.spill, (size_t)t.spill_depth * t.spill_lanes * sizeof(int32_t))) return e;
  QueryArgs a;
  memset(&a, 0, sizeof a);
  a.scene = c.scene;
  a.rays = d_rays;
  a.hits = d_hits;
  a.n = n;
  a.time_lo = sc.flat.time_lo;
  a.time_hi = sc.flat.time_hi;
  a.leaf16 = t.leaf16;
  a.spill_lanes = t.spill_lanes;
  a.spill = static_cast<int32_t*>(c.spill.p);
  a.err = c.err_host;
  return launch_query(var.hit, "hit_kernel launch", resident, k.blk, n, a, stream, ev0, ev1);
}

int enqueue_sample_rays(Scene& sc, DeviceCopy& c, uint64_t n, const void* d_rays, const float* bg, uint32_t max_depth,
                        void* d_samples, hipStream_t stream, hipEvent_t ev0, hipEvent_t ev1) {
  const Knobs kn = read_knobs();
  const Variant var = path_kernel_variant(sc.flat, kn);
  const KernelCfg& k = var.cfg;
  const int resident = resident_blocks(c, GRID_SAMPLE, (const void*)var.sample, k.blk, "sample kernel", kn.verbose);
  const LaunchTuning t = tune_launch(kn, sc.flat, k, resident);
  if (int e = grow(c.spill, (size_t)t.walk.spill_depth * t.walk.spill_lanes * sizeof(int32_t))) return e;
  SampleArgs a;
  memset(&a, 0, sizeof a);
  a.scene = c.scene;
  a.max_depth = max_depth;
  memcpy(a.bg, bg, sizeof a.bg);
  a.time_lo = sc.flat.time_lo;
  a.time_hi = sc.flat.time_hi;
  a.quota16 = t.quota16;
  a.leaf16 = t.walk.leaf16;
  a.regen_min = t.regen_min;
  a.spill_lanes = t.walk.spill_lanes;
  a.spill = static_cast<int32_t*>(c.spill.p);
  a.counters = c.counters;
  a.queue = dispensers(c);
  a.err = c.err_host;
  const uint64_t waves = (uint64_t)resident * (uint32_t)k.blk / 64u;
  HIPCHK(hipMemsetAsync(c.counters, 0, COUNTER_WORDS * sizeof(unsigned long long), stream), "hipMemsetAsync");
  if (ev0) HIPCHK(hipEventRecord(ev0, stream), "hipEventRecord");
  for (uint64_t first = 0; first < n; first += SAMPLE_LAUNCH_MAX) {
    const uint64_t m = std::min(SAMPLE_LAUNCH_MAX, n - first);
    if (first) HIPCHK(hipMemsetAsync(a.queue, 0, DISP * DISP_STRIDE * sizeof(unsigned long long), stream),
                      "hipMemsetAsync(queue)");
    a.rays = static_cast<const char*>(d_rays) + first * sizeof(rtw_ray);
    a.samples = static_cast<char*>(d_samples) + first * sizeof(rtw_sample);
    a.n = (uint32_t)m;
    a.batch = kn.batch.set ? t.batch : pass_batch(t.batch, m, waves);
    const int grid = (int)std::min<uint64_t>((uint64_t)resident, (m + (uint32_t)k.blk - 1u) / (uint32_t)k.blk);
    hipLaunchKernelGGL(var.sample, dim3(grid), dim3(k.blk), 0, stream, a);
    HIPCHK(hipGetLastError(), "sample_kernel launch");
  }
  if (ev1) HIPCHK(hipEventRecord(ev1, stream), "hipEventRecord");
  return RTW_OK;
}

int enqueue_scatter_rays(Scene& sc, DeviceCopy& c, uint64_t n, const void* d_rays, const void* d_hits, const float* bg,
                         void* d_out_rays, void* d_out_scatter, hipStream_t stream, hipEvent_t ev0, hipEvent_t ev1) {
  const Knobs kn = read_knobs();
  ScatterArgs a;
  memset(&a, 0, sizeof a);
  a.scene = c.scene;
  a.mshade = static_cast<const DevShade*>(c.mshade.p);
  a.n_mats = (uint32_t)sc.flat.mshade.size();
  memcpy(a.bg, bg, sizeof a.bg);
  a.rays = d_rays;
  a.hits = d_hits;
  a.out_rays = d_out_rays;
  a.out_scatter = d_out_scatter;
  a.n = n;
  const int resident = resident_blocks(c, GRID_SCATTER, (const void*)dev::scatter_kernel, dev::SHADE_BLOCK,
                                       "scatter_kernel", kn.verbose);
  return launch_query(dev::scatter_kernel, "scatter_kernel launch", resident, dev::SHADE_BLOCK, n, a, stream, ev0, ev1);
}

int enqueue_camera_rays(DeviceCopy& c, const Frame& f, uint64_t first, uint64_t n, void* d_rays, hipStream_t stream,
                        hipEvent_t ev0, hipEvent_t ev1) {
  const Knobs kn = read_knobs();
  const RenderArgs r = frame_args(c, f, TileSet{}, nullptr);
  CameraRaysArgs a;
  memset(&a, 0, sizeof a);
  a.cam = r.cam;
  a.fw1 = r.fw1; a.fh1 = r.fh1; a.rw1 = r.rw1; a.rh1 = r.rh1; a.time_span = r.time_span;
  a.w = f.w; a.spp = f.spp;
  a.row_paths = (uint64_t)f.w * f.spp;
  a.h1 = f.h - 1u;
  a.seed_hash = r.seed_hash;
  a.first = first;
  a.n = n;
  a.rays = d_rays;
  const int resident = resident_blocks(c, GRID_CAMERA, (const void*)dev::camera_rays_kernel, dev::SHADE_BLOCK,
                                       "camera_rays_kernel", kn.verbose);
  return launch_query(dev::camera_rays_kernel, "camera_rays_kernel launch", resident, dev::SHADE_BLOCK, n, a, stream,
                      ev0, ev1);
}

int enqueue_unpack(uint32_t w, uint32_t h, const uint32_t* d_tiles, uint32_t n_tiles, const float* d_packed,
                   float* d_image, hipStream_t stream) {
  const uint32_t n = n_tiles * 64u;
  if (!n) return RTW_OK;
  hipLaunchKernelGGL(dev::unpack_tiles_kernel, dim3((n + 255) / 256), dim3(256), 0, stream, w, h, (w + 7u) / 8u, d_tiles,
                     n_tiles, d_packed, d_image);
  HIPCHK(hipGetLastError(), "unpack_tiles_kernel");
  return RTW_OK;
}

template <class T>
struct DiagBuf {
  T* p = nullptr;
  bool alloc(size_t n) { return hipMalloc((void**)&p, n * sizeof(T)) == hipSuccess; }
  ~DiagBuf() { hipFree(p); }
};

}

using namespace rtw;

extern "C" {

int rtw_diag_libm(int fn, uint32_t n, const float* a, const float* b, float* out) {
  if (fn < 0 || fn > 5 || (n && (!a || !out || ((fn == 3 || fn == 4) && !b)))) return fail(RTW_EINVAL, "bad arguments");
  if (!n) return RTW_OK;
  int ndev = 0;
  if (hipGetDeviceCount(&ndev) != hipSuccess || ndev <= 0) return fail(RTW_ENODEV, "no HIP device visible");
  DiagBuf<float> da, db, dout;
  const size_t bytes = (size_t)n * sizeof(float);
  if (!da.alloc(n) || !dout.alloc(n) || ((fn == 3 || fn == 4) && !db.alloc(n))) return fail(RTW_ENOMEM, "hipMalloc(diag)");
  if (hipMemcpy(da.p, a, bytes, hipMemcpyHostToDevice) != hipSuccess ||
      (db.p && hipMemcpy(db.p, b, bytes, hipMemcpyHostToDevice) != hipSuccess))
    return fail(RTW_ENODEV, "hipMemcpy(diag)");
  hipLaunchKernelGGL(dev::libm_kernel, dim3((n + 255) / 256), dim3(256), 0, nullptr, fn, n, da.p, db.p, dout.p);
  if (hipGetLastError() != hipSuccess || hipMemcpy(out, dout.p, bytes, hipMemcpyDeviceToHost) != hipSuccess)
    return fail(RTW_ENODEV, "libm_kernel");
  return RTW_OK;
}

int rtw_diag_sweep(int fn, uint32_t lo, uint32_t hi, uint64_t* counts, uint32_t* bad, uint32_t cap) {
  if (fn != 0 || lo > hi || !counts || (cap && !bad)) return fail(RTW_EINVAL, "bad arguments");
  int ndev = 0;
  if (hipGetDeviceCount(&ndev) != hipSuccess || ndev <= 0) return fail(RTW_ENODEV, "no HIP device visible");
  DiagBuf<unsigned long long> dn;
  DiagBuf<uint32_t> dbad;
  if (!dn.alloc(3) || !dbad.alloc(cap ? cap : 1)) return fail(RTW_ENOMEM, "hipMalloc(sweep)");
  if (hipMemset(dn.p, 0, 3 * sizeof(unsigned long long)) != hipSuccess) return fail(RTW_ENODEV, "hipMemset(sweep)");
  hipLaunchKernelGGL(dev::sweep_kernel, dim3(16384), dim3(256), 0, nullptr, fn, lo, hi, dn.p, dbad.p, cap);
  unsigned long long h[3];
  if (hipGetLastError() != hipSuccess || hipMemcpy(h, dn.p, sizeof h, hipMemcpyDeviceToHost) != hipSuccess ||
      (cap && hipMemcpy(bad, dbad.p, cap * sizeof(uint32_t), hipMemcpyDeviceToHost) != hipSuccess))
    return fail(RTW_ENODEV, "sweep_kernel");
  counts[0] = h[0];
  counts[1] = h[1];
  return RTW_OK;
}

}
```

raytracer-weekend_amd/csrc/rtw_path_kernel.hpp:

```cpp
#pragma once
#include "rtw_dev_shade.hpp"
#include "rtw_dev_trace.hpp"

namespace rtw {
namespace dev {

constexpr uint32_t BATCH = 2048;

struct PathState {
  Ray ray;
  V3 T;
  uint64_t rng;
  uint32_t pid;
  uint32_t depth;
};

__device__ __forceinline__ uint32_t fastdiv(uint32_t n, uint64_t M) {
  const uint64_t t = (uint64_t)(uint32_t)(M >> 32) * n + __umulhi((uint32_t)M, n);
  return (uint32_t)(t >> 32);
}

__device__ __forceinline__ uint64_t rfl64(uint64_t x) {
  const uint32_t hi = (uint32_t)__builtin_amdgcn_readfirstlane((int)(uint32_t)(x >> 32));
  const uint32_t lo = (uint32_t)__builtin_amdgcn_readfirstlane((int)(uint32_t)x);
  return ((uint64_t)hi << 32) | lo;
}

struct StartArgs {
  DevCamera cam;
  float fw1, fh1, rw1, rh1, time_span;
  uint32_t w, h, spp, max_depth, tiles_x, slot_base, tile_first, tile_stride;
  uint64_t spp_magic, tiles_x_magic, seed_hash;
  const uint32_t* tile_ids;
};
__device__ __forceinline__ void fill_start_args(const RenderArgs& a, StartArgs& o) {
  o.cam = a.cam;
  o.fw1 = a.fw1; o.fh1 = a.fh1; o.rw1 = a.rw1; o.rh1 = a.rh1; o.time_span = a.time_span;
  o.w = a.w; o.h = a.h; o.spp = a.spp; o.max_depth = a.max_depth; o.tiles_x = a.tiles_x;
  o.slot_base = a.slot_base; o.tile_first = a.tile_first; o.tile_stride = a.tile_stride;
  o.spp_magic = a.spp_magic; o.tiles_x_magic = a.tiles_x_magic; o.seed_hash = a.seed_hash;
  o.tile_ids = a.tile_ids;
}

struct StartMade {
  float rdx, rdy;
  V3 d;
  uint64_t rng;
};
template <bool FROM_LDS, bool AB>
__device__ __forceinline__ bool start_make(const StartArgs& a, uint64_t pid, StartMade& m) {
  if constexpr (FROM_LDS) asm volatile("" ::: "memory");
  const uint32_t hi = (uint32_t)(pid >> 6), l = (uint32_t)pid & 63u;
  const uint32_t slot = a.spp > 1u ? fastdiv(hi, a.spp_magic) : hi, s = hi - slot * a.spp;
  const uint32_t gslot = a.slot_base + slot;
  const uint32_t tile = a.tile_ids ? a.tile_ids[gslot] : a.tile_first + gslot * a.tile_stride;
  const uint32_t ty = a.tiles_x > 1u ? fastdiv(tile, a.tiles_x_magic) : tile;
  const uint32_t i = (tile - ty * a.tiles_x) * 8u + (l & 7u), row = ty * 8u + (l >> 3);
  const uint32_t j = a.h - 1u - row;
  const DevCamera& C = a.cam;
  uint64_t rng = xoro_seed(splitmix64(a.seed_hash ^ (((uint64_t)j << 48) | ((uint64_t)i << 32) | s)));
  const float u = div_by_recip((float)i + gen_f32(rng), a.fw1, a.rw1);
  const float v = div_by_recip((float)j + gen_f32(rng), a.fh1, a.rh1);
  const V3 rd = scale(rand_in_unit_disk<AB>(rng), C.lens_radius);
  const V3 off = add(scale(ld3(C.u), rd.x), scale(ld3(C.v), rd.y));
  m.rdx = rd.x;
  m.rdy = rd.y;
  m.d = sub(sub(add(add(ld3(C.llc), scale(ld3(C.horizontal), u)), scale(ld3(C.vertical), v)), ld3(C.origin)), off);
  m.rng = rng;
  return i < a.w && row < a.h;
}
template <bool FENCE, bool AB>
__device__ __forceinline__ void start_take(const StartArgs& a, float rdx, float rdy, uint64_t rng, uint32_t pid,
                                           PathState& st) {
  if constexpr (FENCE) asm volatile("" ::: "memory");
  const DevCamera& C = a.cam;
  const V3 off = add(scale(ld3(C.u), rdx), scale(ld3(C.v), rdy));
  st.ray.o = add(ld3(C.origin), off);
  st.ray.time = gen_range<AB>(rng, C.time0, C.time1, a.time_span);
  st.rng = rng;
  st.T = mk(1.f, 1.f, 1.f);
  st.depth = a.max_depth;
  st.pid = pid;
}

template <bool FROM_LDS, int LST_BLK = 0, int LST_ROW = 0, bool AB = FROM_LDS>
__device__ __forceinline__ bool start_path(const StartArgs& a, uint64_t pid, PathState& st, uint16_t* lst = nullptr) {
  if constexpr (FROM_LDS) asm volatile("" ::: "memory");
  const uint32_t hi = (uint32_t)(pid >> 6), l = (uint32_t)pid & 63u;
  const uint32_t slot = a.spp > 1u ? fastdiv(hi, a.spp_magic) : hi, s = hi - slot * a.spp;
  const uint32_t gslot = a.slot_base + slot;
  const uint32_t tile = a.tile_ids ? a.tile_ids[gslot] : a.tile_first + gslot * a.tile_stride;
  const uint32_t ty = a.tiles_x > 1u ? fastdiv(tile, a.tiles_x_magic) : tile;
  const uint32_t i = (tile - ty * a.tiles_x) * 8u + (l & 7u), row = ty * 8u + (l >> 3);
  if (i >= a.w || row >= a.h) return false;
  const uint32_t j = a.h - 1u - row;
  const DevCamera& C = a.cam;
  uint64_t rng = xoro_seed(splitmix64(a.seed_hash ^ (((uint64_t)j << 48) | ((uint64_t)i << 32) | s)));
  const float u = div_by_recip((float)i + gen_f32(rng), a.fw1, a.rw1);
  const float v = div_by_recip((float)j + gen_f32(rng), a.fh1, a.rh1);
  const V3 rd = scale(rand_in_unit_disk<AB>(rng), C.lens_radius);
  const V3 off = add(scale(ld3(C.u), rd.x), scale(ld3(C.v), rd.y));
  st.ray.o = add(ld3(C.origin), off);
  st.ray.d = sub(sub(add(add(ld3(C.llc), scale(ld3(C.horizontal), u)), scale(ld3(C.vertical), v)), ld3(C.origin)),
                 off);
  st.ray.time = gen_range<AB>(rng, C.time0, C.time1, a.time_span);
  st.rng = rng;
  st.T = mk(1.f, 1.f, 1.f);
  st.depth = a.max_depth;
  st.pid = (uint32_t)pid;
  if constexpr (LST_BLK > 0) {
    const uint32_t v[5] = {0x3F800000u, 0x3F800000u, 0x3F800000u, a.max_depth, (uint32_t)pid};
#pragma unroll
    for (int k = 0; k < 5; ++k) {
      lst[(LST_ROW + 2 * k) * LST_BLK] = (uint16_t)v[k];
      lst[(LST_ROW + 2 * k + 1) * LST_BLK] = (uint16_t)(v[k] >> 16);
    }
  }
  return true;
}

struct KernelCfg {
  int stack;
  bool spill;
  int occ;
  uint32_t feat;
  int blk = BLOCK;
  int ncap = 0;
  bool half = false;
  bool s16 = false;
  constexpr bool lds_nodes() const { return ncap > 0; }
  constexpr bool ldsn_ring() const { return ncap > 0 && blk == 1024 && feat == F_SPHERES; }
  constexpr int lst_rows() const { return s16 ? 10 : 0; }
  constexpr int lst_row0() const { return stack + (s16 ? 1 : 0); }
  constexpr bool lst() const { return lst_rows() > 0; }
  constexpr bool shard() const { return ncap > 0; }
  constexpr bool sring() const { return feat == (F_BOXES | F_LIST) || ldsn_ring(); }
  constexpr int ring_words() const { return ldsn_ring() ? 7 : 10; }
  constexpr bool root_lds() const { return half && s16 && ncap == 0 && RTW_MESH_ROOT > 0; }
  constexpr bool alignbit_draws() const { return !(feat & F_TRI); }
  constexpr bool start_args_in_lds() const { return alignbit_draws() || s16; }
  constexpr uint32_t node_quads() const { return half ? 7u : 8u; }
  constexpr bool codes16_stack() const { return ncap > 0 || s16; }
  constexpr int far_lds_nodes() const { return half ? 0 : ncap; }
  constexpr int stk_words() const { return codes16_stack() ? 1 : (stack + 1) * blk; }
  constexpr int stk16_words(int more = 0) const { return ncap > 0 ? stack * blk : (s16 ? (stack + 1 + more) * blk : 1); }
  constexpr uint32_t lds_node_quads() const {
    return ncap > 0 ? ncap * node_quads() : (root_lds() ? RTW_MESH_ROOT * node_quads() : 1u);
  }
};

template <KernelCfg K>
__device__ __forceinline__ void fill_nodes_lds(const DevScene& S, float4* nodes_lds) {
  if constexpr (K.ncap > 0) {
    const float4* g = K.half ? reinterpret_cast<const float4*>(S.hnodes) : reinterpret_cast<const float4*>(S.nodes);
    for (uint32_t k = threadIdx.x; k < S.n_nodes * K.node_quads(); k += K.blk) nodes_lds[k] = g[k];
  }
  if constexpr (K.root_lds()) {
    const uint32_t nq = min(S.n_nodes, (uint32_t)RTW_MESH_ROOT) * K.node_quads();
    if (threadIdx.x < nq) nodes_lds[threadIdx.x] = reinterpret_cast<const float4*>(S.hnodes)[threadIdx.x];
  }
}

template <bool COUNT, KernelCfg K>
__global__ __launch_bounds__(K.blk) __attribute__((amdgpu_waves_per_eu(K.occ, 8))) void path_kernel(RenderArgs a) {
  __shared__ int32_t stk_all[K.stk_words()];
  __shared__ uint16_t stk16_all[K.stk16_words(K.lst_rows())];
  __shared__ float4 nodes_lds[K.lds_node_quads()];
  fill_nodes_lds<K>(a.scene, nodes_lds);
  __shared__ StartArgs start_lds[K.start_args_in_lds() ? 1 : 0 + 1];
  StartArgs sa_reg;
  if constexpr (K.start_args_in_lds()) {
    if (threadIdx.x == 0) fill_start_args(a, start_lds[0]);
  } else {
    fill_start_args(a, sa_reg);
  }
  const StartArgs& SA = K.start_args_in_lds() ? start_lds[0] : sa_reg;
  __syncthreads();
  uint16_t* stk16 = stk16_all + threadIdx.x;
  int32_t* stk = stk_all + threadIdx.x;
  int32_t* spill = a.spill + (size_t)blockIdx.x * K.blk + threadIdx.x;
  const uint32_t lane = threadIdx.x & 63u;
  constexpr bool LST = K.lst();
  auto lst_st = [&](int k, uint32_t v) {
    stk16[(K.lst_row0() + 2 * k) * K.blk] = (uint16_t)v;
    stk16[(K.lst_row0() + 2 * k + 1) * K.blk] = (uint16_t)(v >> 16);
  };
  auto lst_ld = [&](int k) -> uint32_t {
    return (uint32_t)stk16[(K.lst_row0() + 2 * k) * K.blk] | ((uint32_t)stk16[(K.lst_row0() + 2 * k + 1) * K.blk] << 16);
  };
  const DevScene& S = a.scene;
  const V3 bg = ld3(a.bg);
  const uint64_t P = a.n_paths;
  unsigned long long* const dispenser = a.queue;
  const uint32_t batch = a.batch, ndisp = batch < 1024u ? DISP : 1u;
  const uint64_t NB = (P + batch - 1u) / batch;
  uint32_t cnt[15] = {0, 0, 0, 0, 0, 0, 0, 0, 0, 0, 0, 0, 0, 0, 0};
  unsigned long long nrays = 0;
  __shared__ uint64_t pool_lds[K.blk / 64][K.shard() ? 5 : 3];
  uint64_t* const pool = pool_lds[K.s16 ? __builtin_amdgcn_readfirstlane(threadIdx.x >> 6) : threadIdx.x >> 6];
  if (lane == 0) { pool[0] = 0; pool[1] = 0; }
  if (K.shard() && lane == 0) pool[K.shard() ? 4 : 0] = 0;
  auto refill = [&](uint64_t& b, uint64_t& e) {
    if (lane == 0) {
      uint64_t bb = P, ee = P;
      uint32_t k = (uint32_t)pool[4];
      for (; k < ndisp; ++k) {
        const uint32_t d = (blockIdx.x + k) & (ndisp - 1u);
        const uint64_t g = atomicAdd(dispenser + d * DISP_STRIDE, 1ull) * ndisp + d;
        if (g < NB) {
          bb = g * batch;
          ee = bb + batch < P ? bb + batch : P;
          break;
        }
      }
      pool[2] = bb;
      pool[K.shard() ? 3 : 0] = ee;
      pool[K.shard() ? 4 : 0] = k;
    }
    b = rfl64(pool[2]);
    e = rfl64(pool[K.shard() ? 3 : 0]);
  };
  constexpr uint32_t RW = K.ring_words(), RS = RW * 64u + (K.ldsn_ring() ? 2u : 0u);
  __shared__ uint32_t ring_lds[K.sring() ? (K.blk / 64) * RS : 1];
  __shared__ uint32_t ring_head_lds[K.sring() && !K.ldsn_ring() ? K.blk / 64 : 1];
  if constexpr (K.ldsn_ring()) {
    static_assert(sizeof stk_all + sizeof stk16_all + sizeof nodes_lds + sizeof start_lds + sizeof pool_lds +
                          sizeof ring_lds + sizeof ring_head_lds <= 81920,
                  "the 1024-lane ring kernel's LDS must leave room for 2 workgroups per CU");
  }
  uint32_t* const ring = ring_lds + (K.sring() ? (threadIdx.x >> 6) * RS : 0u);
  uint32_t* const ring_head = K.ldsn_ring() ? ring + RW * 64u : ring_head_lds + (K.sring() ? threadIdx.x >> 6 : 0u);
  uint32_t* const ring_base = ring + (K.ldsn_ring() ? RW * 64u + 1u : 0u);
  if (K.sring() && lane == 0) ring_head[0] = 64u;
  bool exhausted = false;
  bool has = false;
  TraceState ts;
  ts.on = false;
  PathState st;
  st.pid = 0;
  st.rng = 0;
  st.depth = 0;
  uint64_t ph[11] = {0, 0, 0, 0, 0, 0, 0, 0, 0, 0, 0};
  const uint64_t t_start = COUNT ? __builtin_amdgcn_s_memtime() : 0;
  uint64_t t_mark = t_start;
  auto phase = [&](int k) {
    if (COUNT) {
      const uint64_t t = __builtin_amdgcn_s_memtime();
      ph[k] += t - t_mark;
      t_mark = t;
    }
  };
  for (;;) {
    phase(2);
    const uint64_t need = __ballot(!has);
    if constexpr (K.sring()) {
      if (need != 0 && !exhausted && ((uint32_t)__popcll(need) >= a.regen_min || need == __ballot(1))) {
        const uint32_t n_need = (uint32_t)__popcll(need);
        const uint32_t rank =
            __builtin_amdgcn_mbcnt_hi((uint32_t)(need >> 32), __builtin_amdgcn_mbcnt_lo((uint32_t)need, 0u));
        const uint64_t t_sp = COUNT ? __builtin_amdgcn_s_memtime() : 0;
        uint32_t head = (uint32_t)__builtin_amdgcn_readfirstlane((int)ring_head[0]);
        const uint32_t have = 64u - head;
        auto take = [&](uint32_t e) {
          if constexpr (K.ldsn_ring()) {
            const uint32_t lo = ring[5 * 64 + e], hi = ring[6 * 64 + e];
            const float rdx = __uint_as_float(ring[e]), rdy = __uint_as_float(ring[64 + e]);
            st.ray.d = mk(__uint_as_float(ring[2 * 64 + e]), __uint_as_float(ring[3 * 64 + e]),
                          __uint_as_float(ring[4 * 64 + e]));
            start_take<true, K.alignbit_draws()>(SA, rdx, rdy, ((uint64_t)hi << 32) | lo, ring_base[0] + e, st);
            has = (lo | hi) != 0u;
          } else {
            const uint32_t lo = ring[7 * 64 + e], hi = ring[8 * 64 + e];
            st.ray.o = mk(__uint_as_float(ring[e]), __uint_as_float(ring[64 + e]), __uint_as_float(ring[2 * 64 + e]));
            st.ray.d = mk(__uint_as_float(ring[3 * 64 + e]), __uint_as_float(ring[4 * 64 + e]),
                          __uint_as_float(ring[5 * 64 + e]));
            st.ray.time = __uint_as_float(ring[6 * 64 + e]);
            st.rng = ((uint64_t)hi << 32) | lo;
            st.pid = ring[9 * 64 + e];
            st.T = mk(1.f, 1.f, 1.f);
            st.depth = SA.max_depth;
            has = (lo | hi) != 0u;
          }
        };
        const bool first = !has && rank < have;
        if (first) take(head + rank);
        if (n_need > have) {
          uint64_t pool_next = rfl64(pool[0]), pool_end = rfl64(pool[1]);
          if (pool_next >= pool_end) {
            if constexpr (K.shard()) {
              refill(pool_next, pool_end);
            } else {
              if (lane == 0) pool[2] = atomicAdd(dispenser, (unsigned long long)batch);
              const uint64_t b = rfl64(pool[2]);
              pool_next = b < P ? b : P;
              pool_end = b < P ? (b + batch < P ? b + batch : P) : P;
            }
          }
          if (pool_next < pool_end) {
            const uint64_t id = pool_next + lane;
            if constexpr (K.ldsn_ring()) {
              StartMade m;
              const bool ok = start_make<K.start_args_in_lds(), K.alignbit_draws()>(SA, id, m);
              ring[lane] = __float_as_uint(m.rdx);
              ring[64 + lane] = __float_as_uint(m.rdy);
              ring[2 * 64 + lane] = __float_as_uint(m.d.x);
              ring[3 * 64 + lane] = __float_as_uint(m.d.y);
              ring[4 * 64 + lane] = __float_as_uint(m.d.z);
              ring[5 * 64 + lane] = ok ? (uint32_t)m.rng : 0u;
              ring[6 * 64 + lane] = ok ? (uint32_t)(m.rng >> 32) : 0u;
              if (lane == 0) ring_base[0] = (uint32_t)pool_next;
            } else {
              PathState g;
              const bool ok = start_path<K.start_args_in_lds(), 0, 0, K.alignbit_draws()>(SA, id, g);
              ring[lane] = __float_as_uint(g.ray.o.x);
              ring[64 + lane] = __float_as_uint(g.ray.o.y);
              ring[2 * 64 + lane] = __float_as_uint(g.ray.o.z);
              ring[3 * 64 + lane] = __float_as_uint(g.ray.d.x);
              ring[4 * 64 + lane] = __float_as_uint(g.ray.d.y);
              ring[5 * 64 + lane] = __float_as_uint(g.ray.d.z);
              ring[6 * 64 + lane] = __float_as_uint(g.ray.time);
              ring[7 * 64 + lane] = ok ? (uint32_t)g.rng : 0u;
              ring[8 * 64 + lane] = ok ? (uint32_t)(g.rng >> 32) : 0u;
              ring[9 * 64 + lane] = (uint32_t)id;
            }
            pool_next += 64u;
            if (!has && !first) take(rank - have);
            head = n_need - have;
          } else {
            exhausted = true;
            head = 64u;
          }
          if (lane == 0) { pool[0] = pool_next; pool[1] = pool_end; }
        } else {
          head += n_need;
        }
        if (lane == 0) ring_head[0] = head;
        if (COUNT) ph[6] += __builtin_amdgcn_s_memtime() - t_sp;
      }
    } else if (need != 0 && !exhausted && ((uint32_t)__popcll(need) >= a.regen_min || need == __ballot(1))) {
      const uint32_t n_need = (uint32_t)__popcll(need);
      const uint32_t rank =
          __builtin_amdgcn_mbcnt_hi((uint32_t)(need >> 32), __builtin_amdgcn_mbcnt_lo((uint32_t)need, 0u));
      uint64_t pool_next = rfl64(pool[0]), pool_end = rfl64(pool[1]);
      const uint64_t avail = pool_end - pool_next;
      uint64_t nb = P, ne = P;
      if (avail < n_need) {
        if constexpr (K.shard()) {
          uint64_t b, e;
          refill(b, e);
          if (b < e) {
            nb = b;
            ne = e;
          } else {
            exhausted = true;
          }
        } else {
          if (lane == 0) pool[2] = atomicAdd(dispenser, (unsigned long long)batch);
          const uint64_t b = rfl64(pool[2]);
          if (b < P) {
            nb = b;
            ne = b + batch < P ? b + batch : P;
          } else {
            exhausted = true;
          }
        }
      }
      const uint64_t t_sp = COUNT ? __builtin_amdgcn_s_memtime() : 0;
      if (!has) {
        const uint64_t id = rank < avail ? pool_next + rank : nb + (rank - avail);
        if ((rank < avail || id < ne) &&
            start_path<K.start_args_in_lds(), LST ? K.blk : 0, K.lst_row0(), K.alignbit_draws()>(SA, id, st, stk16)) {
          has = true;
        }
      }
      if (COUNT) ph[6] += __builtin_amdgcn_s_memtime() - t_sp;
      if (avail >= n_need) {
        pool_next += n_need;
      } else {
        pool_next = nb + (n_need - avail);
        pool_end = ne;
        if (pool_next > pool_end) pool_next = pool_end;
      }
      if (lane == 0) { pool[0] = pool_next; pool[1] = pool_end; }
    }
    phase(0);
    if (__ballot(has) == 0) {
      if (exhausted) break;
      continue;
    }
    nrays += (unsigned long long)__popcll(__ballot(has && !ts.on));
    if (!has) continue;
    if (!ts.on) {
      trace_begin<COUNT, K.feat, K.stack, K.blk, K.codes16_stack(), K.far_lds_nodes()>(S, st.ray, ts, cnt, st.rng, stk16,
                                                                                       stk, a.err, nodes_lds);
    }
    if (!(K.feat & F_LIST)) {
      const uint32_t act = (uint32_t)__popcll(__ballot(1));
      const uint32_t quota = (act * a.quota16 + 15u) >> 4;
      const uint32_t leaf_thr = (act * a.leaf16 + 15u) >> 4;
      trace_run<COUNT, K.stack, K.spill, K.feat, K.blk, K.ncap, K.half, K.s16>(S, st.ray, ts, stk, spill, a.spill_lanes, cnt,
                                                                              quota, leaf_thr, st.rng, a.err, ph + 4, nodes_lds, stk16);
    } else {
      ts.node = -1;
      ts.sp = 0;
    }
    phase(1);
    __builtin_amdgcn_s_setprio(0);
    if (ts.node >= 0 || ts.sp > 0) continue;
    ts.on = false;
    if (COUNT) simd_tick(cnt, 12, 13);
    const Best b = ts.b;
#ifdef RTW_DIAG_TRACE_PID
    if ((RTW_DIAG_TRACE_PID) < 0 || st.pid == (uint32_t)(RTW_DIAG_TRACE_PID))
      printf("rtwtrace pid %u o %a %a %a d %a %a %a t %a prim %d key %u rng %016llx\n", st.pid, st.ray.o.x, st.ray.o.y,
             st.ray.o.z, st.ray.d.x, st.ray.d.y, st.ray.d.z, b.t, b.prim, b.prim >= 0 ? S.prims[b.prim].key : 0u,
             (unsigned long long)st.rng);
#endif
    bool done = false;
    V3 L = mk(0.f, 0.f, 0.f);
    const V3 T0 = st.T;
    auto path_T = [&]() -> V3 {
      return LST ? mk(__uint_as_float(lst_ld(0)), __uint_as_float(lst_ld(1)), __uint_as_float(lst_ld(2))) : T0;
    };
    if (b.prim < 0) {
      L = mul(path_T(), bg);
      done = true;
      if (__builtin_expect(b.prim == -2, 0)) {
        if constexpr (K.shard()) {
          for (uint32_t d = 0; d < DISP; ++d) atomicMax(dispenser + d * DISP_STRIDE, (unsigned long long)NB);
        } else {
          atomicMax(dispenser, (unsigned long long)P);
        }
        pool[0] = pool[1];
        if constexpr (K.ldsn_ring()) ring_head[0] = 64u;
      }
    } else {
      DevShade sh;
      if constexpr (LST) {
        const float4 q = *reinterpret_cast<const float4*>(S.shade + b.prim);
        sh.kind = __float_as_uint(q.x); sh.param = q.y; sh.a[0] = q.z; sh.a[1] = q.w;
        sh.a[2] = S.shade[b.prim].a[2];
      } else {
        sh = S.shade[b.prim];
      }
      const bool solid_light = (K.feat & F_LIGHT) && (K.feat & F_TRI) && (sh.kind & 0xfffu) == (MT_LIGHT | (SM_SOLID << 8));
      Rec h;
      if (!solid_light) h = hit_record<K.feat>(S, st.ray, b, sh.kind);
      else h = Rec{mk(0.f, 0.f, 0.f), mk(0.f, 0.f, 0.f), 0.0f, 0.0f, true, 0u};
#ifdef RTW_SHADE_DIAG
      phase(7);
#endif
      const MatKind kind = mat_kind<K.feat>(sh.kind);
      V3 rs = mk(0.f, 0.f, 0.f);
      phase(2);
      if (kind.lam || kind.met || kind.iso) rs = rand_in_unit_sphere<K.alignbit_draws()>(st.rng);
      phase(3);
      const V3 ud = unit(kind.lam ? rs : st.ray.d);
      const V3 att = mat_attenuation<K.feat>(S, sh, kind, h, [&] { return ld3(LST ? S.shade[b.prim].b : sh.b); });
#ifdef RTW_SHADE_DIAG
      phase(8);
#endif
      V3 Tn = mk(0.f, 0.f, 0.f);
      if (kind.light) {
        L = mul(path_T(), att);
        done = true;
      } else {
        const V3 dir = mat_direction<K.feat>(sh, kind, h, ud, rs, st.rng, done);
        const V3 Tp = path_T();
        const V3 T2 = mul(Tp, att);
        if (done) L = mul(Tp, mk(0.f, 0.f, 0.f));
        Tn = T2;
        if constexpr (LST) {
          lst_st(0, __float_as_uint(T2.x));
          lst_st(1, __float_as_uint(T2.y));
          lst_st(2, __float_as_uint(T2.z));
        } else {
          st.T = T2;
        }
        st.ray.o = h.p;
        st.ray.d = dir;
      }
// ... 55 lines not shown
```

raytracer-weekend_amd/csrc/rtw_render.cpp:

```cpp
#include <math.h>
#include <string.h>

#include <algorithm>

#include "../../include/rtw.h"
#include "rtw_scene.hpp"

namespace rtw {

template <class T>
static size_t put(std::vector<uint8_t>& blob, const std::vector<T>& v) {
  size_t off = (blob.size() + 255) & ~(size_t)255;
  blob.resize(off + sizeof(T) * v.size());
  if (!v.empty()) memcpy(blob.data() + off, v.data(), sizeof(T) * v.size());
  return off;
}

int upload(Scene& s, int device) {
  int ndev = 0;
  if (hipGetDeviceCount(&ndev) != hipSuccess || ndev <= 0)
    return fail(RTW_ENODEV, "no HIP device visible (the render core has no CPU fallback)");
  const int nlog = s.alias_n > 0 ? s.alias_n : ndev;
  if (device >= nlog) return fail(RTW_EINVAL, "device %d >= device count %d", device, nlog);
  const Flat& f = s.flat;
  std::vector<uint8_t> blob;
  DevFar far = f.far;
  const size_t o_nodes = put(blob, f.nodes4), o_far = put(blob, std::vector<DevFar>{far});
  size_t o_prims = put(blob, f.prims), o_always = put(blob, f.always);
  if (o_prims - o_far != DEVFAR_BACK) return fail(RTW_EINVAL, "internal: far record not %u B before the prims", DEVFAR_BACK);
  reinterpret_cast<DevFar*>(blob.data() + o_far)->nodes_back = (uint32_t)(o_prims - o_nodes);
  size_t o_tsh = put(blob, f.tshade), o_inst = put(blob, f.insts), o_mat = put(blob, f.mats);
  size_t o_tex = put(blob, f.texs), o_texel = put(blob, f.texels), o_perlin = put(blob, f.perlins);
  size_t o_shade = put(blob, f.shade), o_hnodes = put(blob, f.nodes4h), o_groups = put(blob, f.lgroups);
  blob.resize((blob.size() + 255) & ~(size_t)255);
  int d0 = device >= 0 ? device : 0, d1 = device >= 0 ? device + 1 : nlog;
  DeviceGuard g;
  auto fill = [&](DeviceCopy& c, int d) -> int {
    const int phys = s.alias_n > 0 ? 0 : d;
    c.device = d;
    c.phys = phys;
    HIPCHK(hipSetDevice(phys), "hipSetDevice");
    c.bytes = blob.size();
    HIPCHK(hipMalloc(&c.block, c.bytes), "hipMalloc(scene)");
    HIPCHK(hipMemcpy(c.block, blob.data(), c.bytes, hipMemcpyHostToDevice), "hipMemcpy(scene)");
    HIPCHK(hipMalloc((void**)&c.counters, COUNTER_WORDS * sizeof(unsigned long long)), "hipMalloc(counters)");
    HIPCHK(hipHostMalloc((void**)&c.err_host, 64, hipHostMallocMapped | hipHostMallocCoherent), "hipHostMalloc(error word)");
    *(volatile uint32_t*)c.err_host = 0u;
    if (!f.mshade.empty()) {
      if (int e = grow(c.mshade, f.mshade.size() * sizeof(DevShade))) return e;
      HIPCHK(hipMemcpy(c.mshade.p, f.mshade.data(), f.mshade.size() * sizeof(DevShade), hipMemcpyHostToDevice),
             "hipMemcpy(material shading records)");
    }
    uint8_t* base = (uint8_t*)c.block;
    c.scene.nodes = (const DevNode4*)(base + o_nodes);
    c.scene.hnodes = f.nodes4h.empty() ? nullptr : (const DevNode4h*)(base + o_hnodes);
    c.scene.prims = (const DevPrim*)(base + o_prims);
    c.scene.always = (const uint32_t*)(base + o_always);
    c.scene.tshade = (const DevTriShade*)(base + o_tsh);
    c.scene.insts = (const DevInst*)(base + o_inst);
    c.scene.mats = (const DevMat*)(base + o_mat);
    c.scene.texs = (const DevTex*)(base + o_tex);
    c.scene.texels = (const uint8_t*)(base + o_texel);
    c.scene.perlins = (const DevPerlin*)(base + o_perlin);
    c.scene.shade = (const DevShade*)(base + o_shade);
    c.scene.lgroups = (const DevGroup*)(base + o_groups);
    c.scene.n_lgroups = (uint32_t)f.lgroups.size();
    c.scene.n_nodes = (uint32_t)f.nodes4.size();
    c.scene.n_prims = (uint32_t)f.prims.size();
    c.scene.n_always = (uint32_t)f.always.size();
    c.scene.n_insts = (uint32_t)f.insts.size();
    c.scene.msphere_unit = f.msphere_unit;
    c.scene.uni_inst = f.uni_inst;
    c.scene.bvh_tri = f.bvh_tri;
    c.scene.tri_inst = f.tri_inst;
    c.scene.rect_fast = f.rect_fast;
    memcpy(c.scene.uni_off, f.uni_off, sizeof f.uni_off);
    c.scene.far_check = f.far_check;
    return RTW_OK;
  };
  for (int d = d0; d < d1; ++d) {
    s.dev.emplace_back();
    if (int e = fill(s.dev.back(), d)) {
      release(s);
      return e;
    }
  }
  return RTW_OK;
}

static void free_buf(DevBuf& b) {
  if (b.p) hipFree(b.p);
  b.p = nullptr;
  b.cap = 0;
}

void release(Scene& s) {
  for (DeviceCopy& c : s.dev) {
    if (hipSetDevice(c.phys) != hipSuccess) continue;
    if (c.block) hipFree(c.block);
    if (c.counters) hipFree(c.counters);
    if (c.err_host) hipHostFree(c.err_host);
    for (DevBuf* b : {&c.sbuf, &c.spill, &c.image, &c.tiles, &c.packed, &c.gathered, &c.gather_ids, &c.qrays, &c.qhits,
                       &c.mshade, &c.qscatter, &c.qsamples})
      free_buf(*b);
    for (hipEvent_t e : {c.ev[0], c.ev[1], c.gev[0], c.gev[1]})
      if (e) hipEventDestroy(e);
    if (c.stream) hipStreamDestroy(c.stream);
    for (auto& pair : c.kev)
      for (hipEvent_t e : pair)
        if (e) hipEventDestroy(e);
  }
  s.dev.clear();
}

DeviceCopy* find_copy(Scene& s, int device) {
  for (DeviceCopy& c : s.dev)
    if (c.device == device || device < 0) return &c;
  return nullptr;
}

int grow(DevBuf& b, size_t bytes) {
  if (bytes <= b.cap) return RTW_OK;
  free_buf(b);
  HIPCHK(hipMalloc(&b.p, bytes), "hipMalloc(render buffer)");
  b.cap = bytes;
  return RTW_OK;
}

int check_frame(const rtw_scene* s, const Frame& f, bool out) {
  if (!s || !f.cam || !f.bg || !out) return fail(RTW_EINVAL, "NULL argument");
  if (!s->s.committed) return fail(RTW_ESTATE, "scene not committed");
  return check_image_min(f.w, f.h);
}

int check_image_min(uint32_t w, uint32_t h) {
  if (w < 2 || h < 2) return fail(RTW_EINVAL, "image must be at least 2x2 (lib.rs:84-85 divides by w-1, h-1)");
  return RTW_OK;
}

int check_image_max(uint32_t w, uint32_t h) {
  if (w > 65536u || h > 65536u)
    return fail(RTW_EINVAL, "image %ux%u: at most 65536 x 65536 (16-bit pixel coordinates in the path key)", w, h);
  return RTW_OK;
}

int check_shutter(const rtw_camera& cam, const Flat& f) {
  if (cam.time0 < f.time_lo || cam.time1 > f.time_hi)
    return fail(RTW_EINVAL, "camera shutter [%g, %g) outside the committed motion range [%g, %g]", cam.time0, cam.time1,
                f.time_lo, f.time_hi);
  return RTW_OK;
}

DeviceCopy* need_copy(Scene& s, int device, const char* hint) {
  DeviceCopy* c = find_copy(s, device);
  if (c) return c;
  if (hint) fail(RTW_ENODEV, "scene was not committed to device %d%s", device, hint);
  else fail(RTW_ENODEV, "scene has no device copy");
  return nullptr;
}

int copy_events(DeviceCopy& c) {
  for (hipEvent_t& e : c.ev)
    if (int rc = ensure_event(e)) return rc;
  return RTW_OK;
}

float recip_rn(float b) {
  float y = (float)(1.0 / (double)b), best = y;
  double e = fabs(1.0 - (double)y * (double)b);
  for (float c : {nextafterf(y, 0.0f), nextafterf(y, 2.0f)}) {
    const double ec = fabs(1.0 - (double)c * (double)b);
    if (ec < e) { e = ec; best = c; }
  }
  return best;
}

int check_guard(DeviceCopy& c) {
  volatile uint32_t* e = c.err_host;
  if (e && *e) {
    *e = 0u;
    return fail(RTW_EINVAL, "a path kernel on device %d tripped its BVH traversal guard (corrupt tree?): the frame "
                "it rendered is invalid", c.device);
  }
  return RTW_OK;
}

// ... 231 lines not shown
```

raytracer-weekend_amd/csrc/rtw_scene.hpp:

```cpp
#pragma once
#include <hip/hip_runtime_api.h>
#include <stdint.h>

#include <chrono>
#include <string>
#include <vector>

#include "../../include/rtw.h"
#include "rtw_device.hpp"

struct rtw_scene;

namespace rtw {

enum NodeKind : uint32_t {
  NK_LIST,
  NK_BVH,
  NK_TRANSLATE,
  NK_ROTY,
  NK_SPHERE,
  NK_MSPHERE,
  NK_RECT,
  NK_CUBOID,
  NK_TRI,
  NK_MEDIUM,
};

struct Node {
  NodeKind kind;
  std::vector<uint32_t> ch;
  float f[9] = {0, 0, 0, 0, 0, 0, 0, 0, 0};
  uint32_t axis = 0, mat = 0, tri = 0;
  float sin_t = 0.f, cos_t = 1.f;
};

struct TexH {
  uint32_t type = TT_SOLID, odd = 0, even = 0;
  float c[3] = {0, 0, 0};
  float freq = 0.f;
  uint32_t w = 0, h = 0;
  std::vector<uint8_t> img;
  std::vector<float> grad;
  std::vector<uint32_t> perm;
};

struct MatH {
  uint32_t type = MT_LAMBERT, tex = 0;
  float albedo[3] = {0, 0, 0};
  float param = 0.f;
};

struct Flat {
  std::vector<DevNode> nodes;
  std::vector<DevNode4> nodes4;
  uint32_t stack_need = 0;
  bool codes16 = false;
  uint32_t stack_need4 = 0;
  std::vector<DevNode4h> nodes4h;
  std::vector<DevPrim> prims;
  std::vector<DevShade> shade;
  std::vector<DevShade> mshade;
  std::vector<uint32_t> always;
  std::vector<DevTriShade> tshade;
  std::vector<DevInst> insts;
  std::vector<DevMat> mats;
  std::vector<DevTex> texs;
  std::vector<uint8_t> texels;
  std::vector<DevPerlin> perlins;
  uint32_t depth = 0;
  uint32_t features = 0;
  uint32_t msphere_unit = 1;
  uint32_t uni_inst = 0;
  uint32_t rect_fast = 0;
  std::vector<DevGroup> lgroups;
  uint32_t bvh_tri = 0;
  uint32_t tri_inst = 0;
  float uni_off[3] = {0, 0, 0};
  float time_lo = 0.f, time_hi = 1.f;
  uint32_t far_check = 0;
  DevFar far{};
  float far_d0 = 0.f;
};

struct DevBuf {
  void* p = nullptr;
  size_t cap = 0;
};

struct ResidentGrid {
  const void* fn = nullptr;
  int blocks = 0;
};
enum GridSlot { GRID_PATH, GRID_PATH_COUNT, GRID_HIT, GRID_SCATTER, GRID_CAMERA, GRID_SAMPLE, GRID_SLOTS };

struct DeviceCopy {
  int device = -1;
  int phys = -1;
  void* block = nullptr;
  size_t bytes = 0;
  DevScene scene{};
  unsigned long long* counters = nullptr;
  uint32_t* err_host = nullptr;
  DevBuf sbuf;
  DevBuf spill;
  hipEvent_t kev[64][2] = {};
  uint32_t kev_head = 0, kev_count = 0;
  ResidentGrid grids[GRID_SLOTS];
  DevBuf image, tiles, packed, gathered, gather_ids;
  DevBuf qrays, qhits;
  DevBuf mshade;
  DevBuf qscatter;
  DevBuf qsamples;
  hipEvent_t ev[2] = {nullptr, nullptr};
  hipStream_t stream = nullptr;
  hipEvent_t gev[2] = {nullptr, nullptr};
};

struct Scene {
  std::vector<TexH> tex;
  std::vector<MatH> mat;
  std::vector<Node> nodes;
  std::vector<uint32_t> open{0};
  std::vector<float> tri_v, tri_n, tri_uv;
  std::vector<uint8_t> tri_nm, tri_uvm;
  bool committed = false;
  bool flattened = false;
  Flat flat;
  std::vector<DeviceCopy> dev;
  std::vector<float> multi_ms;
  float multi_gather_ms = 0.0f;
  int alias_n = 0;
  Scene() { nodes.push_back(Node{NK_LIST, {}}); }
};

int fail(int code, const char* fmt, ...);
const char* tuning_env(const char* name);

#define HIPCHK(x, what)                                                                        \
  do {                                                                                         \
    hipError_t e_ = (x);                                                                       \
    if (e_ != hipSuccess) return rtw::fail(RTW_ENODEV, "%s: %s", what, hipGetErrorString(e_)); \
  } while (0)
struct DeviceGuard {
  int prev = 0;
  DeviceGuard() { hipGetDevice(&prev); }
  ~DeviceGuard() { hipSetDevice(prev); }
};
inline int ensure_event(hipEvent_t& e) {
  if (!e) HIPCHK(hipEventCreate(&e), "hipEventCreate");
  return RTW_OK;
}
inline hipStream_t abi_stream(void* s) { return (hipStream_t)s; }
inline double ms_since(std::chrono::steady_clock::time_point t0) {
  return std::chrono::duration<double, std::milli>(std::chrono::steady_clock::now() - t0).count();
}

struct Frame {
  const rtw_camera* cam;
  const float* bg;
  uint32_t w, h, spp, max_depth;
  uint64_t seed;
  uint32_t tiles_x() const { return (w + 7u) / 8u; }
  uint64_t tiles() const { return (uint64_t)((w + 7u) / 8u) * ((h + 7u) / 8u); }
  uint64_t paths() const { return (uint64_t)w * h * spp; }
};
struct TileSet {
  const uint32_t* ids = nullptr;
  uint32_t first = 0, stride = 1, n = 0;
  bool packed = false;
};

int flatten(Scene& s);
std::string dump_scene(const Scene& s);
int upload(Scene& s, int device);
void release(Scene& s);
DeviceCopy* find_copy(Scene& s, int device);
int grow(DevBuf& b, size_t bytes);
int check_frame(const rtw_scene* s, const Frame& f, bool out);
int check_image_min(uint32_t w, uint32_t h);
int check_image_max(uint32_t w, uint32_t h);
int check_shutter(const rtw_camera& cam, const Flat& f);
DeviceCopy* need_copy(Scene& s, int device, const char* hint = "");
int copy_events(DeviceCopy& c);
int collect_stats(DeviceCopy& c, hipStream_t stream, hipEvent_t ev0, hipEvent_t ev1, uint64_t paths, rtw_stats* st);
int check_guard(DeviceCopy& c);
float recip_rn(float b);
int64_t selected_kernel_info(const Scene& s, int field);
int enqueue_render(Scene& s, DeviceCopy& c, const Frame& f, const TileSet& tiles, float* d_out, hipStream_t stream,
                   uint32_t flags, hipEvent_t ev0, hipEvent_t ev1);
int enqueue_hit_rays(Scene& s, DeviceCopy& c, uint64_t n, const void* d_rays, void* d_hits, hipStream_t stream,
                     hipEvent_t ev0, hipEvent_t ev1);
int enqueue_scatter_rays(Scene& s, DeviceCopy& c, uint64_t n, const void* d_rays, const void* d_hits, const float* bg,
                         void* d_out_rays, void* d_out_scatter, hipStream_t stream, hipEvent_t ev0, hipEvent_t ev1);
int enqueue_camera_rays(DeviceCopy& c, const Frame& f, uint64_t first, uint64_t n, void* d_rays, hipStream_t stream,
                        hipEvent_t ev0, hipEvent_t ev1);
int enqueue_sample_rays(Scene& s, DeviceCopy& c, uint64_t n, const void* d_rays, const float* bg, uint32_t max_depth,
                        void* d_samples, hipStream_t stream, hipEvent_t ev0, hipEvent_t ev1);
int enqueue_unpack(uint32_t w, uint32_t h, const uint32_t* d_tiles, uint32_t n_tiles, const float* d_packed,
                   float* d_image, hipStream_t stream);

}

struct rtw_scene {
  rtw::Scene s;
};
```

raytracer-weekend_amd/csrc/rtw_variants.hpp:

```cpp
#pragma once
#include <stdio.h>

#include "rtw_path_kernel.hpp"
#include "rtw_query_kernel.hpp"
#include "rtw_sample_kernel.hpp"

namespace rtw {

typedef void (*path_fn)(RenderArgs);
typedef void (*hit_fn)(QueryArgs);
typedef void (*sample_fn)(SampleArgs);
using dev::KernelCfg;
struct Variant {
  path_fn fn[2];
  hit_fn hit;
  sample_fn sample;
  KernelCfg cfg;
};
template <KernelCfg K>
static Variant make_variant() {
  return {{dev::path_kernel<false, K>, dev::path_kernel<true, K>}, dev::hit_kernel<K>, dev::sample_kernel<K>, K};
}
constexpr KernelCfg with_half(KernelCfg k) { k.half = true; return k; }
constexpr KernelCfg with_spill(KernelCfg k) { k.spill = true; return k; }

struct Knob {
  bool set = false;
  int v = 0;
  int get(int dflt) const { return set ? v : dflt; }
};
struct Knobs {
  Knob stack_lds, half_nodes, generic, list_all, list_occ, occ, ldsn_waves, lds_nodes, ldsn_blk, mesh_s16;
  Knob batch, quota16, leaf16, regen_min, pass_log2;
  bool verbose = false;
};

template <uint32_t F> constexpr KernelCfg WALK4{.stack = dev::STACK_LDS, .spill = false, .occ = 4, .feat = F};
template <uint32_t F> constexpr KernelCfg WALK5{.stack = dev::STACK_LDS5, .spill = false, .occ = 5, .feat = F};
template <uint32_t F> constexpr KernelCfg DEEP5{.stack = dev::STACK_DEEP5, .spill = false, .occ = 5, .feat = F};
constexpr KernelCfg SPHERES6{.stack = dev::STACK_LDS5, .spill = false, .occ = 6, .feat = F_SPHERES};
constexpr KernelCfg SPILL_TEST{.stack = 4, .spill = true, .occ = 4, .feat = F_ALL};
constexpr KernelCfg LIST_ALL{.stack = 1, .spill = false, .occ = 5, .feat = F_ALL | F_LIST};
constexpr KernelCfg LIST_BOXES8{.stack = 1, .spill = false, .occ = 8, .feat = F_BOXES | F_LIST};
constexpr KernelCfg LIST_BOXES6{.stack = 1, .spill = false, .occ = 6, .feat = F_BOXES | F_LIST};
constexpr KernelCfg LDSN_224{.stack = 24, .spill = false, .occ = 6, .feat = F_SPHERES, .blk = 512, .ncap = 224};
constexpr KernelCfg LDSN_512{.stack = 16, .spill = false, .occ = 8, .feat = F_SPHERES, .blk = 512, .ncap = 144};
constexpr KernelCfg LDSN_448{.stack = 18, .spill = false, .occ = 7, .feat = F_SPHERES, .blk = 448, .ncap = 160};
constexpr KernelCfg LDSN_1024{.stack = 16, .spill = false, .occ = 8, .feat = F_SPHERES, .blk = 1024, .ncap = 144};
template <uint32_t F>
constexpr KernelCfg S16_7{.stack = dev::STACK_DEEP5, .spill = false, .occ = 7, .feat = F, .s16 = true};
template <uint32_t F>
constexpr KernelCfg S16_6{.stack = dev::STACK_DEEP5, .spill = false, .occ = 6, .feat = F, .s16 = true};

template <uint32_t F>
static Variant pick5(const Knobs& kn, uint32_t need, bool half = false, bool codes16 = false) {
  using namespace dev;
  if constexpr (F == F_MESHES) {
    int s16 = kn.mesh_s16.get(half ? 7 : 0);
    if (s16 != 0 && s16 != 6 && s16 != 7) {
      fprintf(stderr, "rtw: RTW_MESH_S16=%d ignored (0, 6 or 7)\n", s16);
      s16 = half ? 7 : 0;
    }
    if (codes16 && s16 != 0 && need <= (uint32_t)STACK_DEEP5) {
      if (s16 == 7) return half ? make_variant<with_half(S16_7<F>)>() : make_variant<S16_7<F>>();
      return half ? make_variant<with_half(S16_6<F>)>() : make_variant<S16_6<F>>();
    }
  }
  if constexpr (F == F_MESHES) {
    if (half && need <= (uint32_t)STACK_LDS5) return make_variant<with_half(WALK5<F>)>();
    if (half && need <= (uint32_t)STACK_DEEP5) return make_variant<with_half(DEEP5<F>)>();
  }
  if (need <= (uint32_t)STACK_LDS5) return make_variant<WALK5<F>>();
  if constexpr (F == F_MESHES || F == F_ALL) {
    if (need <= (uint32_t)STACK_DEEP5) return make_variant<DEEP5<F>>();
    return make_variant<with_spill(DEEP5<F>)>();
  }
  return make_variant<with_spill(WALK5<F>)>();
}
Variant pick_mesh(const Knobs& kn, uint32_t need, bool half, bool codes16);

}
```

Measured before the change: 26820 Mrays/s.

## Precompute per-tile primary-ray candidate lists via conservative beam culling

Adds a kernel that builds, for each 8x8 tile, a list of up to 15 primitives whose boxes the tile's camera beam (including the lens aperture) may hit. The trace start can then test only those primitives and skip the BVH walk when the list is decided. The lists are cached per camera and resolution and used only when the lens lies inside the far region and the ring LDS variant is selected. It also lowers quota16 when lists are active. This adds a preprocessing kernel, extra buffers and a conservative float/double culling test that must never miss a hit.

```diff
diff --git a/include/rtw.h b/include/rtw.h
--- a/include/rtw.h
+++ b/include/rtw.h
@@ -197,6 +197,10 @@
 int rtw_diag_libm(int fn, uint32_t n, const float* a, const float* b, float* out);
 int rtw_diag_sweep(int fn, uint32_t lo, uint32_t hi, uint64_t* counts, uint32_t* bad, uint32_t cap);
 int rtw_diag_recip(uint32_t n, const float* b, float* out);
+int rtw_diag_tile_lists(rtw_scene* s, int device, const rtw_camera* cam, uint32_t w, uint32_t h, uint32_t* records,
+                        uint64_t cap_words, uint32_t* n_over, uint32_t* prim_keys, uint32_t cap_keys);
+int rtw_diag_tile_beam(const rtw_camera* cam, uint32_t w, uint32_t h, uint32_t tile, const float* box_lo,
+                       const float* box_hi);
 
 int rtw_tonemap(const float* rgb_sum, uint32_t n_pixels, uint32_t spp, uint8_t* rgb8);
 
diff --git a/raytracer-weekend_amd/__init__.py b/raytracer-weekend_amd/__init__.py
--- a/raytracer-weekend_amd/__init__.py
+++ b/raytracer-weekend_amd/__init__.py
@@ -172,6 +172,9 @@
     "rtw_tonemap": (C.c_int, [_F, C.c_uint32, C.c_uint32, _U8]),
     "rtw_diag_libm": (C.c_int, [C.c_int, C.c_uint32, _F, _F, _F]),
     "rtw_diag_recip": (C.c_int, [C.c_uint32, _F, _F]),
+    "rtw_diag_tile_lists": (C.c_int, [C.c_void_p, C.c_int, C.POINTER(rtw_camera), C.c_uint32, C.c_uint32, _U32,
+                                      C.c_uint64, _U32, _U32, C.c_uint32]),
+    "rtw_diag_tile_beam": (C.c_int, [C.POINTER(rtw_camera), C.c_uint32, C.c_uint32, C.c_uint32, _F, _F]),
     "rtw_diag_sweep": (C.c_int, [C.c_int, C.c_uint32, C.c_uint32, C.POINTER(C.c_uint64), _U32, C.c_uint32]),
     "rtw_scene_preset": (C.c_int, [C.c_void_p, C.c_char_p, C.c_float, C.c_uint64, C.c_char_p,
                                    C.POINTER(rtw_camera), _F]),
@@ -680,6 +683,28 @@
     return out
 
 
+def diag_tile_beam(cam, w: int, h: int, tile: int, box_lo, box_hi) -> bool:
+    lo, hi = _fa(box_lo), _fa(box_hi)
+    rc = lib().rtw_diag_tile_beam(C.byref(cam.c), w, h, tile, _fp(lo), _fp(hi))
+    if rc < 0:
+        _check(rc)
+    return bool(rc)
+
+
+def diag_tile_lists(scene, cam, w: int, h: int, device: int = 0):
+    nt = n_tiles(w, h)
+    rec = np.zeros(nt * 8, np.uint32)
+    over = C.c_uint32()
+    keys = np.zeros(65536, np.uint32)
+    n = lib().rtw_diag_tile_lists(scene._p, device, C.byref(cam.c), w, h, _up(rec), rec.size, C.byref(over),
+                                  _up(keys), keys.size)
+    if n < 0:
+        _check(n)
+    half = rec.view(np.uint16).reshape(nt, 16)
+    lists = [None if r[0] == 0xFFFF else [int(x) for x in r[1:1 + int(r[0])]] for r in half]
+    return lists, int(over.value), keys[:n]
+
+
 def tile_partition(w: int, h: int, n_parts: int, part: int):
     nt = n_tiles(w, h)
     per = (nt + n_parts - 1) // n_parts if n_parts > 0 else 0
diff --git a/raytracer-weekend_amd/csrc/rtw.hpp b/raytracer-weekend_amd/csrc/rtw.hpp
--- a/raytracer-weekend_amd/csrc/rtw.hpp
+++ b/raytracer-weekend_amd/csrc/rtw.hpp
@@ -165,6 +165,13 @@
     check(rtw_camera_rays(s_, device, &cam.c, w, h, spp, seed, first, n, rays.data(), st));
     return rays;
   }
+  std::vector<uint32_t> tile_lists(const Camera& cam, uint32_t w, uint32_t h, int device = -1,
+                                   uint32_t* n_over = nullptr) const {
+    std::vector<uint32_t> rec((size_t)((w + 7u) / 8u) * ((h + 7u) / 8u) * 8u);
+    const int n = rtw_diag_tile_lists(s_, device, &cam.c, w, h, rec.data(), rec.size(), n_over, nullptr, 0);
+    if (n < 0) check(n);
+    return rec;
+  }
   std::vector<Scatter> scatter_rays(std::vector<Ray>& rays, const std::vector<Hit>& hits, Color background,
                                     int device = -1, rtw_stats* st = nullptr) const {
     if (rays.size() != hits.size()) throw Error(RTW_EINVAL, "rays and hits differ in length");
diff --git a/raytracer-weekend_amd/csrc/rtw_capi.cpp b/raytracer-weekend_amd/csrc/rtw_capi.cpp
--- a/raytracer-weekend_amd/csrc/rtw_capi.cpp
+++ b/raytracer-weekend_amd/csrc/rtw_capi.cpp
@@ -580,6 +580,7 @@
     case 15: return (int64_t)llround(1000.0 * (double)sc.flat.far_d0);
     case 16: case 17: case 18: case 19: case 20: case 21: case 22: case 23:
       return selected_kernel_info(sc, what - 16);
+    case 24: case 25: return last_render_lists(const_cast<Scene&>(sc), what - 24);
     case 4: return (int64_t)sc.flat.depth;
     case 5: return (int64_t)sc.flat.always.size();
     case 6: return (int64_t)sc.flat.insts.size();
diff --git a/raytracer-weekend_amd/csrc/rtw_dev_trace.hpp b/raytracer-weekend_amd/csrc/rtw_dev_trace.hpp
--- a/raytracer-weekend_amd/csrc/rtw_dev_trace.hpp
+++ b/raytracer-weekend_amd/csrc/rtw_dev_trace.hpp
@@ -219,11 +219,13 @@
 constexpr bool far_kernel_feat(uint32_t feat) {
   return !(feat & F_LIST) && (feat & (F_SPHERE | F_MSPHERE | F_MEDIUM)) && feat != F_MESHES;
 }
-template <bool COUNT, uint32_t FEAT, int STACK = 1, int BLK = BLOCK, bool C16 = false, int NCAP = 0>
+template <bool COUNT, uint32_t FEAT, int STACK = 1, int BLK = BLOCK, bool C16 = false, int NCAP = 0, bool RING = false>
 __device__ __forceinline__ void trace_begin(const DevScene& S, const Ray& r, TraceState& ts, uint32_t* cnt,
                                             uint64_t seg, uint16_t* stk16 = nullptr, int32_t* stk = nullptr,
-                                            uint32_t* err = nullptr, const float4* lnodes = nullptr) {
+                                            uint32_t* err = nullptr, const float4* lnodes = nullptr,
+                                            int32_t start = -3) {
   ts.b = Best{INFINITY, 0u, -1, 0.0f, 0.0f};
+  const bool decided = RING && start != -3;
   constexpr bool RECT_LIST = (FEAT & F_LIST) && (FEAT & F_RECT) && !(FEAT & (F_SPHERE | F_MSPHERE | F_TRI | F_MEDIUM));
   if constexpr (RECT_LIST) {
     trace_rect_list<COUNT>(S, r, ts.b, cnt);
@@ -239,6 +241,15 @@
         cur = inst;
       }
       test_prim<COUNT, FEAT, true, true>(S, pi, lr, ts.b, cnt, seg);
+    }
+  } else if constexpr (RING) {
+    const SphRcp rq = sph_rcp(r);
+    const uint32_t n = decided ? (start >= 0 ? 1u : 0u) : S.n_always;
+    for (uint32_t k = 0; __any(k < n); ++k) {
+      if (k < n) {
+        const uint32_t pi = decided ? (uint32_t)start : uload(S.always + k);
+        test_prim<COUNT, FEAT, false, false>(S, pi, r, ts.b, cnt, seg, &rq);
+      }
     }
   } else {
     constexpr bool SPH_ONLY = (FEAT & (F_RECT | F_TRI | F_MEDIUM | F_INST)) == 0 && (FEAT & (F_SPHERE | F_MSPHERE));
@@ -267,7 +278,7 @@
       const float ty = fabsf(r.o.y - mid.y) + half.y;
       const float tz = fabsf(r.o.z - mid.z) + half.z;
       const float D2 = tx * tx + ty * ty + tz * tz;
-      const bool far = D2 > mid.w;
+      const bool far = D2 > mid.w && !decided;
       if (__any(far)) {
         bool need = false;
         float delta = 0.0f;
@@ -299,7 +310,7 @@
   } else {
     asm volatile("" : "+v"(root));
   }
-  ts.node = walk ? root : -1;
+  ts.node = (walk && !decided) ? root : -1;
   ts.pend = 0;
   ts.sp = 0;
   ts.on = true;
diff --git a/raytracer-weekend_amd/csrc/rtw_device.hpp b/raytracer-weekend_amd/csrc/rtw_device.hpp
--- a/raytracer-weekend_amd/csrc/rtw_device.hpp
+++ b/raytracer-weekend_amd/csrc/rtw_device.hpp
@@ -200,6 +200,9 @@
   int32_t* spill;
   uint32_t spill_depth;
   uint32_t spill_lanes;
-};
+  const uint32_t* tile_lists;
+};
+
+constexpr uint32_t TILE_LIST_WORDS = 8, TILE_LIST_MAX = 15, TILE_LIST_OVER = 0xFFFFu;
 
 }
diff --git a/raytracer-weekend_amd/csrc/rtw_flatten.cpp b/raytracer-weekend_amd/csrc/rtw_flatten.cpp
--- a/raytracer-weekend_amd/csrc/rtw_flatten.cpp
+++ b/raytracer-weekend_amd/csrc/rtw_flatten.cpp
@@ -734,6 +734,10 @@
     f.depth = bb.max_depth;
   }
   for (const Leaf& L : rest) f.prims.push_back(L.p);
+  f.pboxes.clear();
+  for (const Leaf& L : rest)
+    f.pboxes.insert(f.pboxes.end(), {L.wbox.lo[0], L.wbox.lo[1], L.wbox.lo[2], 0.0f, L.wbox.hi[0], L.wbox.hi[1],
+                                     L.wbox.hi[2], 0.0f});
   for (const Leaf& L : huge) {
     f.always.push_back((uint32_t)f.prims.size());
     f.prims.push_back(L.p);
diff --git a/raytracer-weekend_amd/csrc/rtw_kernel.hip b/raytracer-weekend_amd/csrc/rtw_kernel.hip
--- a/raytracer-weekend_amd/csrc/rtw_kernel.hip
+++ b/raytracer-weekend_amd/csrc/rtw_kernel.hip
@@ -10,6 +10,7 @@
 #include "rtw_scene.hpp"
 #include "rtw_variants.hpp"
 #include "rtw_shade_kernel.hpp"
+#include "rtw_tile_beam.h"
 
 namespace rtw {
 namespace dev {
@@ -48,6 +49,51 @@
   const uint32_t i = (tile % tiles_x) * 8u + (lane & 7u), row = (tile / tiles_x) * 8u + (lane >> 3);
   if (i >= w || row >= h) return;
   for (int c = 0; c < 3; ++c) img[((size_t)row * w + i) * 3 + c] = packed[(size_t)g * 3 + c];
+}
+
+constexpr uint32_t TILE_LIST_BLOCK = 64, TILE_LIST_CHUNK = 256;
+struct TileListArgs {
+  DevCamera cam;
+  uint32_t w, h, n_tiles, n_bvh, cap;
+  const float4* boxes;
+  uint32_t* lists;
+  uint32_t* n_over;
+};
+__global__ __launch_bounds__(TILE_LIST_BLOCK) void tile_list_kernel(TileListArgs a) {
+  __shared__ BeamBox cbox[TILE_LIST_CHUNK];
+  const uint32_t tile = blockIdx.x * TILE_LIST_BLOCK + threadIdx.x;
+  const BeamCamera C = beam_camera(a.cam.origin, a.cam.u, a.cam.v, a.cam.llc, a.cam.horizontal, a.cam.vertical,
+                                   a.cam.lens_radius);
+  const BeamTile T = beam_tile(C, a.w, a.h, tile < a.n_tiles ? tile : 0u);
+  uint32_t rec[TILE_LIST_WORDS] = {0, 0, 0, 0, 0, 0, 0, 0};
+  uint32_t n = 0;
+  for (uint32_t base = 0; base < a.n_bvh; base += TILE_LIST_CHUNK) {
+    const uint32_t m = min(TILE_LIST_CHUNK, a.n_bvh - base);
+    __syncthreads();
+    for (uint32_t k = threadIdx.x; k < m; k += TILE_LIST_BLOCK) {
+      const float4 lo = a.boxes[2u * (base + k)], hi = a.boxes[2u * (base + k) + 1u];
+      const float l[3] = {lo.x, lo.y, lo.z}, h[3] = {hi.x, hi.y, hi.z};
+      cbox[k] = beam_box(C, l, h);
+    }
+    __syncthreads();
+    for (uint32_t k = 0; k < m; ++k) {
+      if (beam_may_hit(C, T, cbox[k])) {
+        ++n;
+        if (n <= TILE_LIST_MAX) {
+          const uint32_t v = (base + k) << ((n & 1u) * 16u);
+#pragma unroll
+          for (uint32_t q = 0; q < TILE_LIST_WORDS; ++q) rec[q] |= (n >> 1) == q ? v : 0u;
+        }
+      }
+    }
+  }
+  if (tile >= a.n_tiles) return;
+  const bool over = n > a.cap;
+  rec[0] = over ? TILE_LIST_OVER : (rec[0] | n);
+  uint4* o = reinterpret_cast<uint4*>(a.lists + (size_t)tile * TILE_LIST_WORDS);
+  o[0] = make_uint4(rec[0], rec[1], rec[2], rec[3]);
+  o[1] = make_uint4(rec[4], rec[5], rec[6], rec[7]);
+  if (over) atomicAdd(a.n_over, 1u);
 }
 
 __global__ void libm_kernel(int fn, uint32_t n, const float* a, const float* b, float* out) {
@@ -118,6 +164,8 @@
   k.leaf16 = knob("RTW_LEAF16");
   k.regen_min = knob("RTW_REGEN_MIN");
   k.pass_log2 = knob("RTW_PASS_LOG2");
+  k.tile_lists = knob("RTW_TILE_LISTS");
+  k.tile_list_cap = knob("RTW_TILE_LIST_CAP");
   const char* v = getenv("RTW_VERBOSE");
   k.verbose = v && atoi(v);
   return k;
@@ -183,6 +231,18 @@
   const KernelCfg k = path_kernel_variant(s.flat, read_knobs()).cfg;
   const int64_t v[8] = {k.stack, k.spill, k.occ, k.feat, k.blk, k.ncap, k.half, k.s16};
   return field >= 0 && field < 8 ? v[field] : -1;
+}
+
+int64_t last_render_lists(Scene& s, int field) {
+  DeviceCopy* c = find_copy(s, -1);
+  if (!c) return 0;
+  if (field == 0 || !c->lists_used) return field == 0 ? (int64_t)c->lists_used : 0;
+  DeviceGuard g;
+  uint32_t n = 0;
+  if (hipSetDevice(c->phys) != hipSuccess || hipDeviceSynchronize() != hipSuccess ||
+      hipMemcpy(&n, c->lists_count, sizeof n, hipMemcpyDeviceToHost) != hipSuccess)
+    return -1;
+  return (int64_t)n;
 }
 
 static int resident_blocks(DeviceCopy& c, GridSlot slot, const void* fn, int block, const char* what, bool verbose) {
@@ -318,6 +378,7 @@
     a.slot_base = base;
     a.n_paths = (uint64_t)ns * per_slot;
     a.batch = kn.batch.set ? t.batch : pass_batch(t.batch, a.n_paths, waves);
+    if (!kn.quota16.set) a.quota16 = (a.tile_lists && a.batch == t.batch) ? 8u : t.quota16;
     if (base) HIPCHK(hipMemsetAsync(a.queue, 0, DISP * DISP_STRIDE * sizeof(unsigned long long), stream),
                      "hipMemsetAsync(queue)");
     hipEvent_t* ke = c.kev[c.kev_head];
@@ -335,6 +396,61 @@
   return RTW_OK;
 }
 
+static bool lens_is_near(const Flat& flat, const rtw_camera& cam) {
+  if (!flat.far_check) return false;
+  const DevFar& F = flat.far;
+  const double R = fabs((double)cam.lens_radius);
+  for (int q = 0; q < 4; ++q) {
+    double D2 = 0.0;
+    for (int k = 0; k < 3; ++k) {
+      const double o = (double)cam.origin[k] + ((q & 1) ? R : -R) * (double)cam.u[k] + ((q & 2) ? R : -R) * (double)cam.v[k];
+      const double t = fabs(o - (double)F.mid[k]) + (double)F.half[k];
+      D2 += t * t;
+    }
+    if (!(D2 * (1.0 + 1.0e-6) <= (double)F.d2)) return false;
+  }
+  return true;
+}
+
+static dev::TileListArgs tile_list_args(const rtw_camera& cam, uint32_t w, uint32_t h, uint32_t n_bvh, uint32_t cap) {
+  dev::TileListArgs t;
+  memset(&t, 0, sizeof t);
+  memcpy(t.cam.origin, cam.origin, sizeof t.cam.origin);
+  memcpy(t.cam.llc, cam.lower_left_corner, sizeof t.cam.llc);
+  memcpy(t.cam.horizontal, cam.horizontal, sizeof t.cam.horizontal);
+  memcpy(t.cam.vertical, cam.vertical, sizeof t.cam.vertical);
+  memcpy(t.cam.u, cam.u, sizeof t.cam.u);
+  memcpy(t.cam.v, cam.v, sizeof t.cam.v);
+  t.cam.lens_radius = cam.lens_radius;
+  t.w = w;
+  t.h = h;
+  t.n_tiles = (uint32_t)(((uint64_t)(w + 7u) / 8u) * ((h + 7u) / 8u));
+  t.n_bvh = n_bvh;
+  t.cap = cap;
+  return t;
+}
+
+static int enqueue_tile_lists(Scene& sc, DeviceCopy& c, const rtw_camera& cam, uint32_t w, uint32_t h, uint32_t cap,
+                              uint32_t* lists, uint32_t* n_over, hipStream_t stream) {
+  dev::TileListArgs t = tile_list_args(cam, w, h, sc.flat.far.n_bvh, cap);
+  t.boxes = static_cast<const float4*>(c.pboxes.p);
+  t.lists = lists;
+  t.n_over = n_over;
+  HIPCHK(hipMemsetAsync(n_over, 0, sizeof(uint32_t), stream), "hipMemsetAsync(tile-list counter)");
+  hipLaunchKernelGGL(dev::tile_list_kernel, dim3((t.n_tiles + dev::TILE_LIST_BLOCK - 1u) / dev::TILE_LIST_BLOCK),
+                     dim3(dev::TILE_LIST_BLOCK), 0, stream, t);
+  HIPCHK(hipGetLastError(), "tile_list_kernel launch");
+  return RTW_OK;
+}
+static bool tile_lists_on(const Scene& sc, const DeviceCopy& c, const rtw_camera& cam, uint32_t* cap) {
+  const Knobs kn = read_knobs();
+  *cap = (uint32_t)std::min((int)TILE_LIST_MAX, std::max(1, kn.tile_list_cap.get((int)TILE_LIST_MAX)));
+  const uint32_t n_bvh = sc.flat.far.n_bvh;
+  return kn.tile_lists.get(1) != 0 && path_kernel_variant(sc.flat, kn).cfg.ldsn_ring() && c.pboxes.p &&
+         c.lists_count && n_bvh > 0 && n_bvh < TILE_LIST_OVER && sc.flat.pboxes.size() == (size_t)n_bvh * 8u &&
+         lens_is_near(sc.flat, cam);
+}
+
 int enqueue_render(Scene& sc, DeviceCopy& c, const Frame& f, const TileSet& ts, float* d_out, hipStream_t stream,
                    uint32_t flags, hipEvent_t ev0, hipEvent_t ev1) {
   if (int e = check_guard(c)) return e;
@@ -342,12 +458,31 @@
   if (int e = check_shutter(*f.cam, sc.flat)) return e;
   RenderArgs a = frame_args(c, f, ts, d_out);
   const Knobs kn = read_knobs();
+  c.lists_used = 0;
   HIPCHK(hipMemsetAsync(c.counters, 0, COUNTER_WORDS * sizeof(unsigned long long), stream), "hipMemsetAsync");
   if (ev0) HIPCHK(hipEventRecord(ev0, stream), "hipEventRecord");
   if (ts.n && (f.spp == 0 || f.max_depth == 0)) {
     size_t n = a.packed_out ? (size_t)ts.n * 64 * 3 : (size_t)f.w * f.h * 3;
     HIPCHK(hipMemsetAsync(d_out, 0, n * sizeof(float), stream), "hipMemsetAsync(out)");
   } else if (ts.n) {
+    uint32_t cap = 0;
+    c.lists_used = tile_lists_on(sc, c, *f.cam, &cap) ? 1u : 0u;
+    if (c.lists_used) {
+      DeviceCopy::ListsKey& key = c.lists_key;
+      const bool same = key.valid && key.w == f.w && key.h == f.h && key.cap == cap && key.stream == stream &&
+                        memcmp(&key.cam, f.cam, sizeof key.cam) == 0;
+      if (!same) {
+        key.valid = false;
+        if (int e = grow(c.tile_lists, (size_t)f.tiles() * TILE_LIST_WORDS * sizeof(uint32_t))) return e;
+        if (int e = enqueue_tile_lists(sc, c, *f.cam, f.w, f.h, cap, static_cast<uint32_t*>(c.tile_lists.p),
+                                       c.lists_count, stream))
+          return e;
+        key.cam = *f.cam;
+        key.w = f.w; key.h = f.h; key.cap = cap; key.stream = stream;
+        key.valid = true;
+      }
+      a.tile_lists = static_cast<const uint32_t*>(c.tile_lists.p);
+    }
     if (int e = run_passes(sc, c, a, kn, ts.n, flags & RTW_FLAG_COUNT_TRAVERSAL, stream)) return e;
   }
   if (ev1) HIPCHK(hipEventRecord(ev1, stream), "hipEventRecord");
@@ -499,6 +634,44 @@
   return RTW_OK;
 }
 
+int rtw_diag_tile_lists(rtw_scene* s, int device, const rtw_camera* cam, uint32_t w, uint32_t h, uint32_t* records,
+                        uint64_t cap_words, uint32_t* n_over, uint32_t* prim_keys, uint32_t cap_keys) {
+  if (!s || !cam || !records) return fail(RTW_EINVAL, "NULL argument");
+  if (!s->s.committed) return fail(RTW_ESTATE, "scene not committed");
+  if (int e = check_image_min(w, h)) return e;
+  if (int e = check_image_max(w, h)) return e;
+  DeviceCopy* c = need_copy(s->s, device);
+  if (!c) return RTW_ENODEV;
+  const uint32_t n_bvh = s->s.flat.far.n_bvh;
+  if (!c->pboxes.p || n_bvh == 0 || n_bvh >= TILE_LIST_OVER || s->s.flat.pboxes.size() != (size_t)n_bvh * 8u)
+    return fail(RTW_EINVAL, "the scene has no sphere BVH of under %u primitives: no tile lists", TILE_LIST_OVER);
+  const uint64_t words = (uint64_t)((w + 7u) / 8u) * ((h + 7u) / 8u) * TILE_LIST_WORDS;
+  if (cap_words < words) return fail(RTW_EINVAL, "records: %llu words needed", (unsigned long long)words);
+  const Knobs kn = read_knobs();
+  const uint32_t cap = (uint32_t)std::min((int)TILE_LIST_MAX, std::max(1, kn.tile_list_cap.get((int)TILE_LIST_MAX)));
+  DeviceGuard g;
+  HIPCHK(hipSetDevice(c->phys), "hipSetDevice");
+  DiagBuf<uint32_t> lists, over;
+  if (!lists.alloc(words) || !over.alloc(1)) return fail(RTW_ENOMEM, "hipMalloc(tile lists)");
+  if (int e = enqueue_tile_lists(s->s, *c, *cam, w, h, cap, lists.p, over.p, nullptr)) return e;
+  uint32_t no = 0;
+  if (hipMemcpy(records, lists.p, words * sizeof(uint32_t), hipMemcpyDeviceToHost) != hipSuccess ||
+      hipMemcpy(&no, over.p, sizeof no, hipMemcpyDeviceToHost) != hipSuccess)
+    return fail(RTW_ENODEV, "tile_list_kernel");
+  if (n_over) *n_over = no;
+  for (uint32_t k = 0; prim_keys && k < std::min(cap_keys, n_bvh); ++k) prim_keys[k] = s->s.flat.prims[k].key;
+  return (int)n_bvh;
+}
+
+int rtw_diag_tile_beam(const rtw_camera* cam, uint32_t w, uint32_t h, uint32_t tile, const float* box_lo,
+                       const float* box_hi) {
+  if (!cam || !box_lo || !box_hi) return fail(RTW_EINVAL, "NULL argument");
+  if (int e = check_image_min(w, h)) return e;
+  const BeamCamera C = beam_camera(cam->origin, cam->u, cam->v, cam->lower_left_corner, cam->horizontal, cam->vertical,
+                                   cam->lens_radius);
+  return beam_may_hit(C, beam_tile(C, w, h, tile), beam_box(C, box_lo, box_hi)) ? 1 : 0;
+}
+
 int rtw_diag_sweep(int fn, uint32_t lo, uint32_t hi, uint64_t* counts, uint32_t* bad, uint32_t cap) {
   if (fn != 0 || lo > hi || !counts || (cap && !bad)) return fail(RTW_EINVAL, "bad arguments");
   int ndev = 0;
diff --git a/raytracer-weekend_amd/csrc/rtw_path_kernel.hpp b/raytracer-weekend_amd/csrc/rtw_path_kernel.hpp
--- a/raytracer-weekend_amd/csrc/rtw_path_kernel.hpp
+++ b/raytracer-weekend_amd/csrc/rtw_path_kernel.hpp
@@ -44,9 +44,12 @@
 
 struct StartMade {
   float rdx, rdy;
+  float u, v;
   V3 d;
   uint64_t rng;
+  uint32_t tile;
 };
+constexpr int32_t START_MISS = -1, START_WALK = -3;
 template <bool FROM_LDS, bool AB>
 __device__ __forceinline__ bool start_make(const StartArgs& a, uint64_t pid, StartMade& m) {
   if constexpr (FROM_LDS) asm volatile("" ::: "memory");
@@ -65,22 +68,53 @@
   const V3 off = add(scale(ld3(C.u), rd.x), scale(ld3(C.v), rd.y));
   m.rdx = rd.x;
   m.rdy = rd.y;
+  m.u = u;
+  m.v = v;
+  m.tile = tile;
   m.d = sub(sub(add(add(ld3(C.llc), scale(ld3(C.horizontal), u)), scale(ld3(C.vertical), v)), ld3(C.origin)), off);
   m.rng = rng;
   return i < a.w && row < a.h;
 }
 template <bool FENCE, bool AB>
-__device__ __forceinline__ void start_take(const StartArgs& a, float rdx, float rdy, uint64_t rng, uint32_t pid,
-                                           PathState& st) {
+__device__ __forceinline__ void start_take(const StartArgs& a, float rdx, float rdy, float u, float v, uint64_t rng,
+                                           uint32_t pid, PathState& st) {
   if constexpr (FENCE) asm volatile("" ::: "memory");
   const DevCamera& C = a.cam;
   const V3 off = add(scale(ld3(C.u), rdx), scale(ld3(C.v), rdy));
   st.ray.o = add(ld3(C.origin), off);
+  st.ray.d = sub(sub(add(add(ld3(C.llc), scale(ld3(C.horizontal), u)), scale(ld3(C.vertical), v)), ld3(C.origin)), off);
   st.ray.time = gen_range<AB>(rng, C.time0, C.time1, a.time_span);
   st.rng = rng;
   st.T = mk(1.f, 1.f, 1.f);
   st.depth = a.max_depth;
   st.pid = pid;
+}
+
+template <bool COUNT, uint32_t FEAT, bool AB>
+__device__ __forceinline__ int32_t start_decide(const DevScene& S, const StartArgs& a, const uint32_t* lists,
+                                                const StartMade& m, uint32_t* cnt) {
+  if (!lists) return START_WALK;
+  const uint32_t tile = (uint32_t)__builtin_amdgcn_readfirstlane((int)m.tile);
+  if (tile >= a.tiles_x * ((a.h + 7u) >> 3)) return START_WALK;
+  const uint32_t* const rec = lists + (size_t)tile * TILE_LIST_WORDS;
+  const uint32_t w0 = uload(rec);
+  const uint32_t n = w0 & 0xFFFFu;
+  if (n == TILE_LIST_OVER) return START_WALK;
+  const DevCamera& C = a.cam;
+  Ray r;
+  const V3 off = add(scale(ld3(C.u), m.rdx), scale(ld3(C.v), m.rdy));
+  r.o = add(ld3(C.origin), off);
+  r.d = m.d;
+  uint64_t g = m.rng;
+  r.time = gen_range<AB>(g, C.time0, C.time1, a.time_span);
+  const SphRcp rq = sph_rcp(r);
+  Best b = Best{INFINITY, 0u, -1, 0.0f, 0.0f};
+  for (uint32_t k = 0; k < S.n_always; ++k) test_prim<COUNT, FEAT, false, true>(S, uload(S.always + k), r, b, cnt, g, &rq);
+  for (uint32_t k = 1; k <= n; ++k) {
+    const uint32_t pi = (uload(rec + (k >> 1)) >> ((k & 1u) * 16u)) & 0xFFFFu;
+    test_prim<COUNT, FEAT, false, true>(S, pi, r, b, cnt, g, &rq);
+  }
+  return b.prim;
 }
 
 template <bool FROM_LDS, int LST_BLK = 0, int LST_ROW = 0, bool AB = FROM_LDS>
@@ -234,6 +268,7 @@
   if (K.sring() && lane == 0) ring_head[0] = 64u;
   bool exhausted = false;
   bool has = false;
+  int32_t start_win = START_WALK;
   TraceState ts;
   ts.on = false;
   PathState st;
@@ -265,9 +300,10 @@
           if constexpr (K.ldsn_ring()) {
             const uint32_t lo = ring[5 * 64 + e], hi = ring[6 * 64 + e];
             const float rdx = __uint_as_float(ring[e]), rdy = __uint_as_float(ring[64 + e]);
-            st.ray.d = mk(__uint_as_float(ring[2 * 64 + e]), __uint_as_float(ring[3 * 64 + e]),
-                          __uint_as_float(ring[4 * 64 + e]));
-            start_take<true, K.alignbit_draws()>(SA, rdx, rdy, ((uint64_t)hi << 32) | lo, ring_base[0] + e, st);
+            start_take<true, K.alignbit_draws()>(SA, rdx, rdy, __uint_as_float(ring[2 * 64 + e]),
+                                                 __uint_as_float(ring[3 * 64 + e]), ((uint64_t)hi << 32) | lo,
+                                                 ring_base[0] + e, st);
+            start_win = (int32_t)ring[4 * 64 + e];
             has = (lo | hi) != 0u;
           } else {
             const uint32_t lo = ring[7 * 64 + e], hi = ring[8 * 64 + e];
@@ -301,11 +337,12 @@
             if constexpr (K.ldsn_ring()) {
               StartMade m;
               const bool ok = start_make<K.start_args_in_lds(), K.alignbit_draws()>(SA, id, m);
+              const int32_t win = start_decide<COUNT, K.feat, K.alignbit_draws()>(S, SA, a.tile_lists, m, cnt);
               ring[lane] = __float_as_uint(m.rdx);
               ring[64 + lane] = __float_as_uint(m.rdy);
-              ring[2 * 64 + lane] = __float_as_uint(m.d.x);
-              ring[3 * 64 + lane] = __float_as_uint(m.d.y);
-              ring[4 * 64 + lane] = __float_as_uint(m.d.z);
+              ring[2 * 64 + lane] = __float_as_uint(m.u);
+              ring[3 * 64 + lane] = __float_as_uint(m.v);
+              ring[4 * 64 + lane] = (uint32_t)win;
               ring[5 * 64 + lane] = ok ? (uint32_t)m.rng : 0u;
               ring[6 * 64 + lane] = ok ? (uint32_t)(m.rng >> 32) : 0u;
               if (lane == 0) ring_base[0] = (uint32_t)pool_next;
@@ -390,13 +427,22 @@
     }
     nrays += (unsigned long long)__popcll(__ballot(has && !ts.on));
     if (!has) continue;
+    bool decided = false;
     if (!ts.on) {
-      trace_begin<COUNT, K.feat, K.stack, K.blk, K.codes16_stack(), K.far_lds_nodes()>(S, st.ray, ts, cnt, st.rng, stk16,
-                                                                                       stk, a.err, nodes_lds);
+      if constexpr (K.ldsn_ring()) {
+        decided = start_win != START_WALK;
+        trace_begin<COUNT, K.feat, K.stack, K.blk, K.codes16_stack(), K.far_lds_nodes(), true>(
+            S, st.ray, ts, cnt, st.rng, stk16, stk, a.err, nodes_lds, start_win);
+        start_win = START_WALK;
+      } else {
+        trace_begin<COUNT, K.feat, K.stack, K.blk, K.codes16_stack(), K.far_lds_nodes()>(S, st.ray, ts, cnt, st.rng, stk16,
+                                                                                         stk, a.err, nodes_lds);
+      }
     }
     if (!(K.feat & F_LIST)) {
       const uint32_t act = (uint32_t)__popcll(__ballot(1));
-      const uint32_t quota = (act * a.quota16 + 15u) >> 4;
+      const uint32_t ndec = K.ldsn_ring() ? (uint32_t)__popcll(__ballot(decided)) : 0u;
+      const uint32_t quota = (((act - ndec) * a.quota16 + 15u) >> 4) + ndec;
       const uint32_t leaf_thr = (act * a.leaf16 + 15u) >> 4;
       trace_run<COUNT, K.stack, K.spill, K.feat, K.blk, K.ncap, K.half, K.s16>(S, st.ray, ts, stk, spill, a.spill_lanes, cnt,
                                                                               quota, leaf_thr, st.rng, a.err, ph + 4, nodes_lds, stk16);
diff --git a/raytracer-weekend_amd/csrc/rtw_render.cpp b/raytracer-weekend_amd/csrc/rtw_render.cpp
--- a/raytracer-weekend_amd/csrc/rtw_render.cpp
+++ b/raytracer-weekend_amd/csrc/rtw_render.cpp
@@ -51,6 +51,12 @@
       HIPCHK(hipMemcpy(c.mshade.p, f.mshade.data(), f.mshade.size() * sizeof(DevShade), hipMemcpyHostToDevice),
              "hipMemcpy(material shading records)");
     }
+    if (!f.pboxes.empty()) {
+      if (int e = grow(c.pboxes, f.pboxes.size() * sizeof(float))) return e;
+      HIPCHK(hipMemcpy(c.pboxes.p, f.pboxes.data(), f.pboxes.size() * sizeof(float), hipMemcpyHostToDevice),
+             "hipMemcpy(primitive boxes)");
+    }
+    HIPCHK(hipMalloc((void**)&c.lists_count, 64), "hipMalloc(tile-list counter)");
     uint8_t* base = (uint8_t*)c.block;
     c.scene.nodes = (const DevNode4*)(base + o_nodes);
     c.scene.hnodes = f.nodes4h.empty() ? nullptr : (const DevNode4h*)(base + o_hnodes);
@@ -100,8 +106,9 @@
     if (c.block) hipFree(c.block);
     if (c.counters) hipFree(c.counters);
     if (c.err_host) hipHostFree(c.err_host);
+    if (c.lists_count) hipFree(c.lists_count);
     for (DevBuf* b : {&c.sbuf, &c.spill, &c.image, &c.tiles, &c.packed, &c.gathered, &c.gather_ids, &c.qrays, &c.qhits,
-                       &c.mshade, &c.qscatter, &c.qsamples})
+                       &c.mshade, &c.qscatter, &c.qsamples, &c.pboxes, &c.tile_lists})
       free_buf(*b);
     for (hipEvent_t e : {c.ev[0], c.ev[1], c.gev[0], c.gev[1]})
       if (e) hipEventDestroy(e);
diff --git a/raytracer-weekend_amd/csrc/rtw_scene.hpp b/raytracer-weekend_amd/csrc/rtw_scene.hpp
--- a/raytracer-weekend_amd/csrc/rtw_scene.hpp
+++ b/raytracer-weekend_amd/csrc/rtw_scene.hpp
@@ -61,6 +61,7 @@
   std::vector<DevShade> shade;
   std::vector<DevShade> mshade;
   std::vector<uint32_t> always;
+  std::vector<float> pboxes;
   std::vector<DevTriShade> tshade;
   std::vector<DevInst> insts;
   std::vector<DevMat> mats;
@@ -111,6 +112,16 @@
   DevBuf mshade;
   DevBuf qscatter;
   DevBuf qsamples;
+  DevBuf pboxes;
+  DevBuf tile_lists;
+  uint32_t lists_used = 0, lists_overflow = 0;
+  uint32_t* lists_count = nullptr;
+  struct ListsKey {
+    rtw_camera cam;
+    uint32_t w = 0, h = 0, cap = 0;
+    hipStream_t stream = nullptr;
+    bool valid = false;
+  } lists_key;
   hipEvent_t ev[2] = {nullptr, nullptr};
   hipStream_t stream = nullptr;
   hipEvent_t gev[2] = {nullptr, nullptr};
@@ -186,6 +197,7 @@
 int check_guard(DeviceCopy& c);
 float recip_rn(float b);
 int64_t selected_kernel_info(const Scene& s, int field);
+int64_t last_render_lists(Scene& s, int field);
 int enqueue_render(Scene& s, DeviceCopy& c, const Frame& f, const TileSet& tiles, float* d_out, hipStream_t stream,
                    uint32_t flags, hipEvent_t ev0, hipEvent_t ev1);
 int enqueue_hit_rays(Scene& s, DeviceCopy& c, uint64_t n, const void* d_rays, void* d_hits, hipStream_t stream,
diff --git a/raytracer-weekend_amd/csrc/rtw_tile_beam.h b/raytracer-weekend_amd/csrc/rtw_tile_beam.h
--- /dev/null
+++ b/raytracer-weekend_amd/csrc/rtw_tile_beam.h
@@ -0,0 +1,149 @@
+#pragma once
+#include <math.h>
+#include <stdint.h>
+
+#if defined(__HIPCC__)
+#define RTW_BEAM_HD __host__ __device__ __forceinline__
+#else
+#define RTW_BEAM_HD static inline
+#endif
+
+namespace rtw {
+
+constexpr double BEAM_MARGIN = 2.5e-4;
+
+struct BeamCamera {
+  double ex[3], ey[3], ez[3];
+  double a[3];
+  double l[3], hz[3], vt[3];
+  double mag;
+  double org[3];
+  bool ok;
+};
+
+RTW_BEAM_HD double beam_dot(const double a[3], const double b[3]) { return a[0] * b[0] + a[1] * b[1] + a[2] * b[2]; }
+
+RTW_BEAM_HD BeamCamera beam_camera(const float origin[3], const float u[3], const float v[3], const float llc[3],
+                                   const float horizontal[3], const float vertical[3], float lens_radius) {
+  BeamCamera c;
+  double o[3], lu[3], lv[3], ll[3], hh[3], vv[3], z[3], x[3];
+  for (int k = 0; k < 3; ++k) {
+    o[k] = origin[k]; lu[k] = u[k]; lv[k] = v[k]; hh[k] = horizontal[k]; vv[k] = vertical[k];
+    ll[k] = (double)llc[k] - o[k];
+    c.org[k] = o[k];
+  }
+  for (int k = 0; k < 3; ++k) z[k] = ll[k] + 0.5 * hh[k] + 0.5 * vv[k];
+  const double zn = sqrt(beam_dot(z, z));
+  for (int k = 0; k < 3; ++k) c.ez[k] = z[k] / zn;
+  const double hz = beam_dot(hh, c.ez);
+  for (int k = 0; k < 3; ++k) x[k] = hh[k] - hz * c.ez[k];
+  const double xn = sqrt(beam_dot(x, x));
+  for (int k = 0; k < 3; ++k) c.ex[k] = x[k] / xn;
+  c.ey[0] = c.ez[1] * c.ex[2] - c.ez[2] * c.ex[1];
+  c.ey[1] = c.ez[2] * c.ex[0] - c.ez[0] * c.ex[2];
+  c.ey[2] = c.ez[0] * c.ex[1] - c.ez[1] * c.ex[0];
+  const double R = fabs((double)lens_radius);
+  const double* E[3] = {c.ex, c.ey, c.ez};
+  double m = R;
+  for (int k = 0; k < 3; ++k) {
+    c.a[k] = R * (fabs(beam_dot(lu, E[k])) + fabs(beam_dot(lv, E[k])));
+    c.l[k] = beam_dot(ll, E[k]);
+    c.hz[k] = beam_dot(hh, E[k]);
+    c.vt[k] = beam_dot(vv, E[k]);
+    m = fmax(m, fmax(fabs(o[k]), fmax(fabs((double)llc[k]), fmax(fabs(hh[k]), fabs(vv[k])))));
+  }
+  c.mag = m;
+  c.ok = zn > 0.0 && xn > 0.0 && zn < INFINITY && xn < INFINITY && m < INFINITY;
+  return c;
+}
+
+struct BeamTile {
+  double f0[3], f1[3];
+  double r11, r10, r00, r01;
+  bool ok;
+};
+
+RTW_BEAM_HD BeamTile beam_tile(const BeamCamera& c, uint32_t w, uint32_t h, uint32_t tile) {
+  BeamTile t;
+  const uint32_t tiles_x = (w + 7u) / 8u;
+  const uint32_t tx = tile % tiles_x, ty = tile / tiles_x;
+  const double i0 = 8.0 * tx, i1 = i0 + 8.0;
+  const double j1 = (double)h - 8.0 * ty, j0 = j1 - 8.0;
+  const double pw = 1.0e-3 + 1.0e-5 * i1, ph = 1.0e-3 + 1.0e-5 * fabs(j1);
+  const double su0 = (i0 - pw) / ((double)w - 1.0), su1 = (i1 + pw) / ((double)w - 1.0);
+  const double sv0 = (j0 - ph) / ((double)h - 1.0), sv1 = (j1 + ph) / ((double)h - 1.0);
+  for (int k = 0; k < 3; ++k) {
+    const double h0 = c.hz[k] * su0, h1 = c.hz[k] * su1, v0 = c.vt[k] * sv0, v1 = c.vt[k] * sv1;
+    t.f0[k] = c.l[k] + fmin(h0, h1) + fmin(v0, v1);
+    t.f1[k] = c.l[k] + fmax(h0, h1) + fmax(v0, v1);
+  }
+  const double az = c.a[2];
+  t.ok = c.ok && t.f0[2] - az > 1.0e-9 * (fabs(t.f0[2]) + az);
+  t.r11 = 1.0 / (t.f1[2] - az);
+  t.r10 = 1.0 / (t.f1[2] + az);
+  t.r00 = 1.0 / (t.f0[2] + az);
+  t.r01 = 1.0 / (t.f0[2] - az);
+  return t;
+}
+
+struct BeamBox {
+  double lo[3], hi[3], mag;
+};
+RTW_BEAM_HD BeamBox beam_box(const BeamCamera& c, const float lo[3], const float hi[3]) {
+  BeamBox b;
+  const double* E[3] = {c.ex, c.ey, c.ez};
+  b.mag = 0.0;
+  for (int k = 0; k < 3; ++k) b.mag = fmax(b.mag, fmax(fabs((double)lo[k]), fabs((double)hi[k])));
+  for (int k = 0; k < 3; ++k) {
+    double mid = 0.0, ext = 0.0;
+    for (int j = 0; j < 3; ++j) {
+      const double cj = 0.5 * ((double)lo[j] + (double)hi[j]) - c.org[j], hj = 0.5 * ((double)hi[j] - (double)lo[j]);
+      mid += cj * E[k][j];
+      ext += fabs(hj * E[k][j]);
+    }
+    b.lo[k] = mid - ext;
+    b.hi[k] = mid + ext;
+  }
+  return b;
+}
+
+RTW_BEAM_HD double beam_hi(const BeamCamera& c, const BeamTile& T, int k, double t) {
+  return t * T.f1[k] + fabs(1.0 - t) * c.a[k];
+}
+RTW_BEAM_HD double beam_lo(const BeamCamera& c, const BeamTile& T, int k, double t) {
+  return t * T.f0[k] - fabs(1.0 - t) * c.a[k];
+}
+
+RTW_BEAM_HD bool beam_may_hit(const BeamCamera& c, const BeamTile& T, const BeamBox& b) {
+  if (!T.ok) return true;
+  const double az = c.a[2];
+  const double mag = fmax(c.mag, b.mag);
+  double m = BEAM_MARGIN * 2.0 * mag;
+  double t1 = 0.0;
+  for (int pass = 0; pass < 2; ++pass) {
+    const double z1 = b.hi[2] + m;
+    if (z1 < -az) return false;
+    t1 = (z1 + az) * T.r00;
+    if (t1 > 1.0) t1 = (z1 - az) * T.r01;
+    t1 = t1 * (1.0 + 1.0e-9) + 1.0e-12;
+    if (pass == 0) m = BEAM_MARGIN * (2.0 + t1) * mag;
+  }
+  const double z0 = b.lo[2] - m;
+  double t0 = 0.0;
+  if (z0 > az) {
+    t0 = (z0 - az) * T.r11;
+    if (t0 > 1.0) t0 = (z0 + az) * T.r10;
+    t0 = t0 * (1.0 - 1.0e-9) - 1.0e-12;
+    if (t0 < 0.0) t0 = 0.0;
+  }
+  if (t0 > t1) return false;
+  for (int k = 0; k < 2; ++k) {
+    const double up = fmax(beam_hi(c, T, k, t0), beam_hi(c, T, k, t1));
+    const double dn = fmin(beam_lo(c, T, k, t0), beam_lo(c, T, k, t1));
+    if (b.lo[k] - m > up) return false;
+    if (b.hi[k] + m < dn) return false;
+  }
+  return true;
+}
+
+}
diff --git a/raytracer-weekend_amd/csrc/rtw_variants.hpp b/raytracer-weekend_amd/csrc/rtw_variants.hpp
--- a/raytracer-weekend_amd/csrc/rtw_variants.hpp
+++ b/raytracer-weekend_amd/csrc/rtw_variants.hpp
@@ -32,6 +32,7 @@
 struct Knobs {
   Knob stack_lds, half_nodes, generic, list_all, list_occ, occ, ldsn_waves, lds_nodes, ldsn_blk, mesh_s16;
   Knob batch, quota16, leaf16, regen_min, pass_log2;
+  Knob tile_lists, tile_list_cap;
   bool verbose = false;
 };
 
```

Measured after the change: 28750 Mrays/s (median of 6 runs). +7.2%, better.
